# kakaobrain/rq-vae-transformer

Hardware: NVIDIA H100
Metric: 256x256 images/sec (ImageNet 1.4B RQ-Transformer, 8x8x4 codes, K=16384, top-k 1024, sample+decode) (higher is better)
Workload: dtype fp16

## Files before the change

### include/rqb200.h

```cpp
#ifndef RQB200_H
#define RQB200_H

#include <stddef.h>
#include <stdint.h>

#ifdef __cplusplus
extern "C" {
#endif

#define RQB200_OK 0
#define RQB200_EINVAL (-1)
#define RQB200_ECUDA (-2)
#define RQB200_ENODEV (-3)
#define RQB200_EWORKSPACE (-4)
#define RQB200_ESTATE (-5)

#define RQB200_F32 0
#define RQB200_BF16 1
#define RQB200_F16 2
#define RQB200_E4M3 3

#define RQB200_MODE_EXACT 0
#define RQB200_MODE_FAST 1

#define RQB200_AR_NO_GRAPH 1
#define RQB200_AR_NO_PDL 2
#define RQB200_AR_TRACE 4
#define RQB200_AR_SEQUENTIAL_PREFILL 32

const char* rqb200_last_error(void);
int rqb200_version(void);
int rqb200_device_count(void);

int rqb200_rq_quantize(const float* x, const float* codebook, int64_t N, int K, int C, int D, int64_t* codes,
                       float* quant_list, float* residual_out, void* stream);
int rqb200_rq_quantize_depthwise(const float* x, const float* const* codebooks_host, const int32_t* K_host, int64_t N, int C, int D,
                                 int64_t* codes, float* quant_list, float* residual_out, void* stream);

int rqb200_rq_soft_codes(const float* residual, const float* codebook, int64_t N, int K, int C, float temp, float* soft_out,
                         float* logits_out, void* stream);

int rqb200_rq_embed_sum(const int64_t* codes, const float* codebook, int64_t N, int D, int K, int C, float* out,
                        void* stream);
int rqb200_rq_embed_depth(const int64_t* codes, const float* codebook, int64_t N, int D, int K, int C, float* out,
                          void* stream);
int rqb200_rq_embed_sum_depthwise(const int64_t* codes, const float* const* codebooks_host, const int32_t* K_host, int64_t N, int D,
                                  int C, float* out, void* stream);
int rqb200_rq_embed_depth_depthwise(const int64_t* codes, const float* const* codebooks_host, const int32_t* K_host, int64_t N,
                                    int D, int C, float* out, void* stream);

int rqb200_sample_logits(const float* logits, const float* q, int B, int V, float temperature, int top_k,
                         float top_p, int64_t* out_idx, void* stream);

typedef struct rqb200_block_weights {
    const void *wqkv, *wproj, *w1, *w2;
    const float *bqkv, *bproj, *b1, *b2;
    const float *ln1_w, *ln1_b, *ln2_w, *ln2_b;
    const float *sqkv, *sproj, *s1, *s2;
} rqb200_block_weights;

typedef struct rqb200_ar_config {
    int32_t embed_dim, n_head, n_body, n_head_layers;
    int32_t vocab, H, W, D;
    int32_t vocab_cond, cond_len;
    int32_t code_dim, codebook_size;
    int32_t mode;
    int32_t weight_dtype;
    int32_t flags;
    int32_t split_qkv, split_proj, split_fc1, split_fc2;
    int32_t codebook_per_depth;
    int32_t embed_variant;
} rqb200_ar_config;

#define RQB200_EMB_TOK_INPUT 1
#define RQB200_EMB_TOK_HEAD 2
#define RQB200_EMB_NO_CUMSUM 4
#define RQB200_EMB_TUPLE 8
#define RQB200_EMB_CLS_PER_DEPTH 16

typedef struct rqb200_ar_weights {
    const float *pos_emb_cond, *pos_emb_hw, *pos_emb_d;
    const float* cond_emb;
    const void *w_in, *w_head, *w_cls;
    const float *b_in, *b_head, *b_cls;
    const float *cls_ln_w, *cls_ln_b;
    const float* codebook;
    const rqb200_block_weights* body;
    const rqb200_block_weights* head;
    const void* w_ccls;
    const float *b_ccls, *ccls_ln_w, *ccls_ln_b;
    const float* tok_emb;
    const float *s_in, *s_head, *s_cls, *s_ccls;
} rqb200_ar_weights;

typedef struct rqb200_ar rqb200_ar;

rqb200_ar* rqb200_ar_create(const rqb200_ar_config* cfg, const rqb200_ar_weights* w);
void rqb200_ar_destroy(rqb200_ar* h);
size_t rqb200_ar_workspace_bytes(const rqb200_ar* h, int B);

int rqb200_ar_sample(rqb200_ar* h, const int64_t* partial, const int64_t* cond, int B, int start_h, int start_w,
                     float temperature, const int32_t* top_k_host, const float* top_p_host, const float* noise,
                     int64_t noise_stride, float* logits_out, const int64_t* force_codes, int64_t* out_codes,
                     void* workspace, size_t workspace_bytes, void* stream);
int rqb200_ar_sample_span(rqb200_ar* h, const int64_t* partial, const int64_t* cond, int B, int idx_begin, int idx_end, int resume,
                          float temperature, const int32_t* top_k_host, const float* top_p_host, const float* noise,
                          int64_t noise_stride, float* logits_out, const int64_t* force_codes, int64_t* out_codes,
                          void* workspace, size_t workspace_bytes, void* stream);
int rqb200_ar_sample_span_cfg(rqb200_ar* h, const int64_t* partial, const int64_t* cond, int B, int idx_begin, int idx_end, int resume,
                              float temperature, const int32_t* top_k_host, const float* top_p_host, const float* noise,
                              int64_t noise_stride, float* logits_out, const int64_t* force_codes, int64_t* out_codes,
                              void* workspace, size_t workspace_bytes, void* stream, float cfg_scale);
int rqb200_ar_sample_span_keep(rqb200_ar* h, const int64_t* partial, const int64_t* cond, int B, int idx_begin, int idx_end, int resume,
                               float temperature, const int32_t* top_k_host, const float* top_p_host, const float* noise,
                               int64_t noise_stride, float* logits_out, const int64_t* force_codes, int64_t* out_codes,
                               void* workspace, size_t workspace_bytes, void* stream, const uint8_t* keep, const uint8_t* sampled_host,
                               int cfg_n, float cfg_scale);
int rqb200_ar_step(rqb200_ar* h, const int64_t* xs, int64_t xs_batch_stride, const int64_t* cond, int B, int pos_h, int pos_w,
                   int d, int restart, float* logits_out, void* workspace, size_t workspace_bytes, void* stream);
size_t rqb200_ar_forward_workspace_bytes(const rqb200_ar* h, int B);
int rqb200_ar_forward(rqb200_ar* h, const int64_t* codes, const int64_t* cond, int B, float* logits_out, float* cond_logits_out,
                      void* workspace, size_t workspace_bytes, void* stream);
size_t rqb200_ar_log_prob_workspace_bytes(const rqb200_ar* h, int B);
int rqb200_ar_log_prob(rqb200_ar* h, const int64_t* codes, const int64_t* cond, int B, float* logp_out, float* cond_logp_out,
                       void* workspace, size_t workspace_bytes, void* stream);
int rqb200_ar_trace(rqb200_ar* h, long long* out_host, int cap_launches, char* names, int names_cap);
int64_t rqb200_ar_last_launches(const rqb200_ar* h);

#define RQB200_VAE_NO_GN_FUSE 0x100
typedef struct rqb200_vae_config {
    int32_t ch, n_levels, ch_mult[8], num_res_blocks;
    int32_t n_attn_res, attn_resolutions[8];
    int32_t resolution, z_channels, embed_dim, in_channels, out_ch;
    int32_t codebook_size, depth;
    int32_t mode;
} rqb200_vae_config;

typedef struct rqb200_vae rqb200_vae;

rqb200_vae* rqb200_vae_create(const rqb200_vae_config* cfg);
void rqb200_vae_destroy(rqb200_vae* h);
int rqb200_vae_set_tensor(rqb200_vae* h, const char* key, const void* ptr, int dtype, int64_t numel);
int rqb200_vae_finalize(rqb200_vae* h);
size_t rqb200_vae_workspace_bytes(const rqb200_vae* h, int B);
int rqb200_vae_decode(rqb200_vae* h, const float* z_q, int B, float* out, void* workspace, size_t workspace_bytes,
                      void* stream);
int rqb200_vae_decode_code(rqb200_vae* h, const int64_t* codes, int B, float* out, void* workspace,
                           size_t workspace_bytes, void* stream);
int rqb200_vae_encode(rqb200_vae* h, const float* x, int B, float* z_e, void* workspace, size_t workspace_bytes,
                      void* stream);
int64_t rqb200_vae_last_launches(const rqb200_vae* h);

int rqb200_dbg_gemm_tc(const void* W16, const void* X16, const float* bias, const float* residual, void* out,
                       int out_is_16, int gelu, float* partial, int N_out, int K, int B, int splits, int fmt, void* stream);
int rqb200_dbg_gemm_tc_fp8(const void* W8_packed, const float* scale, const void* X16, const float* bias, const float* residual,
                           void* out, int out_is_16, int gelu, float* partial, int N_out, int K, int B, int splits, void* stream);

int rqb200_dbg_rq_quantize(int form, const float* x, const float* codebook, int64_t N, int K, int C, int D, int64_t* codes,
                           float* quant_list, float* residual_out, void* stream);
int rqb200_dbg_rq_quantize_depthwise(int form, const float* x, const float* const* codebooks_host, const int32_t* K_host, int64_t N,
                                     int C, int D, int64_t* codes, float* quant_list, float* residual_out, void* stream);
int rqb200_dbg_sample_logits(int algo, const float* logits, const float* q, int B, int V, float temperature, int top_k,
                             float top_p, int64_t* out_idx, void* stream);

int rqb200_dbg_conv_tc(const void* X16, const void* W16, const void* X16lo, const void* W16lo, const float* bias,
                       const float* residual, float* out, int B, int H, int W, int Cin, int Cout, int ks, int out_nchw,
                       void* stream);

int rqb200_dbg_conv_tc_gn(const void* X16, const void* W16, const void* X16lo, const void* W16lo, const float* bias,
                          const float* residual, float* out, double* gn_part, int B, int H, int W, int Cin, int Cout, int ks,
                          int out_nchw, void* stream);

int rqb200_dbg_rows_gemm(const void* X16, const void* W16, const float* bias, const float* residual, float* out_f32, void* out_16,
                         int gelu, int fmt, int64_t M, int N_out, int K, void* stream);

int rqb200_dbg_log_prob_rows(const float* logits, int64_t ld, int V, int64_t rows, const int64_t* targets, float* out, void* stream);

int rqb200_dbg_attn_step(int form, const float* part, int S, const float* bqkv, void* kc, void* vc, void* att, int B, int E, int Tmax,
                         const int* t_dev, int t_host, int fmt, void* stream);
int rqb200_dbg_prefill_attn(const void* qkv, void* kc, void* vc, void* att, int G, int T, int E, int Tmax, int fmt, void* stream);
int rqb200_dbg_append_attn(const void* qkv, void* kc, void* vc, void* att, int G, int T0, int T, int E, int Tmax, int fmt, void* stream);
int rqb200_dbg_ln(int form, const float* x_in, const float* part, int S, const float* bias, const float* extra, float* x_out, const float* g,
                  const float* b, void* xn, int64_t rows, int E, int fmt, void* stream);
int rqb200_dbg_act_reduce(const float* part, int S, const float* bias, void* h, int B, int N, int fmt, void* stream);

int rqb200_dbg_vae_conv(const float* X, const void* Wt, int wdtype, const float* bias, const float* residual, float* out, int B, int H,
                        int W, int Cin, int Cout, int ks, int stride, int upsample, int in_nchw, int out_nchw, void* stream);
int rqb200_dbg_groupnorm(int form, const float* X, const float* gamma, const float* beta, float* Y, void* Y16, void* Y16lo,
                         double* stats_ws, int64_t ws_doubles, int B, int HW, int C, int silu, void* stream);
int rqb200_dbg_cast_f16(const float* X, void* Y16, void* Y16lo, int B, int H, int W, int C, int upsample, void* stream);
int rqb200_dbg_vae_attn(const float* qkv, float* out, int B, int HW, int C, void* stream);

#ifdef __cplusplus
}
#endif
#endif
```

### rq-vae-transformer_b200/csrc/conv_tc.cu

```cuda
#include <cstdlib>

#include "kernels.h"
#include "tc_common.cuh"

namespace rqb {

struct ConvTcParams {
    int B, H, W, Cin, Cout;
    int ks;
    int stride;
    int TW, TH, NB;
    int tiles_x, tiles_y, tiles_b, n_tiles_n;
    const float* bias;
    const float* residual;
    float* out;
    int out_nchw;
    void* out16;
    int gelu, fmt;
    int64_t m_rows;
    double* gn_part;
    int gn_chunks;
};

constexpr int CT_THREADS = 288;
constexpr int CT_A_BYTES = 128 * 64 * 2;

template <int CG>
__device__ __forceinline__ void gn_chunk_stats(const float (&wv)[16], bool valid, int lane, float& tot, int& vidx, bool& writer) {
    constexpr int NG = 16 / CG, NV = 2 * NG;
    float vals[NV];
#pragma unroll
    for (int g = 0; g < NG; g++) {
        float s1 = 0.f, s2 = 0.f;
#pragma unroll
        for (int i = 0; i < CG; i++) {
            const float x = valid ? wv[g * CG + i] : 0.f;
            s1 += x;
            s2 = fmaf(x, x, s2);
        }
        vals[g] = s1;
        vals[NG + g] = s2;
    }
    int n = NV;
    vidx = 0;
    int keep_mask = 31;
#pragma unroll
    for (int S = 16; S >= 1; S >>= 1) {
        if (n > 1) {
            const int half = n >> 1;
            const bool up = (lane & S) != 0;
#pragma unroll
            for (int i = 0; i < NV / 2; i++)
                if (i < half) {
                    const float send = up ? vals[i] : vals[i + half];
                    const float keep = up ? vals[i + half] : vals[i];
                    vals[i] = keep + __shfl_xor_sync(0xffffffffu, send, S);
                }
            vidx += up ? half : 0;
            keep_mask &= ~S;
            n = half;
        } else {
            vals[0] += __shfl_xor_sync(0xffffffffu, vals[0], S);
        }
    }
    tot = vals[0];
    writer = (lane & keep_mask) == 0;
}

__device__ __forceinline__ void ct_epilogue16(const ConvTcParams& p, const float (&v)[16], int n0, int q, int lane, int tx, int ty, int tb,
                                              int b, int y, int x, int64_t pix, bool valid) {
    if (n0 >= p.Cout) return;
    if (p.out_nchw) {
        if (!valid) return;
#pragma unroll
        for (int i = 0; i < 16; i++) {
            const int n = n0 + i;
            if (n < p.Cout) p.out[(((int64_t)b * p.Cout + n) * p.H + y) * p.W + x] = v[i] + p.bias[n];
        }
    } else if (p.out16 != nullptr) {
        if (!valid) return;
        float w[16];
#pragma unroll
        for (int i = 0; i < 16; i += 4) {
            const float4 bb = *reinterpret_cast<const float4*>(p.bias + n0 + i);
            w[i] = v[i] + bb.x; w[i + 1] = v[i + 1] + bb.y; w[i + 2] = v[i + 2] + bb.z; w[i + 3] = v[i + 3] + bb.w;
        }
        if (p.gelu) {
#pragma unroll
            for (int i = 0; i < 16; i++) w[i] = gelu_erf(w[i]);
        }
        uint4 pk[2];
        uint32_t* pw = reinterpret_cast<uint32_t*>(pk);
#pragma unroll
        for (int i = 0; i < 8; i++) pw[i] = pack_h16x2(w[2 * i], w[2 * i + 1], p.fmt);
        uint4* o16 = reinterpret_cast<uint4*>(reinterpret_cast<h16*>(p.out16) + pix * p.Cout + n0);
        o16[0] = pk[0];
        o16[1] = pk[1];
    } else {
        float* o = p.out + pix * p.Cout + n0;
        const float* rs = p.residual ? p.residual + pix * p.Cout + n0 : nullptr;
        float wv[16];
#pragma unroll
        for (int i = 0; i < 16; i += 4) {
            float4 bb = *reinterpret_cast<const float4*>(p.bias + n0 + i);
            float4 w = make_float4(v[i] + bb.x, v[i + 1] + bb.y, v[i + 2] + bb.z, v[i + 3] + bb.w);
            if (rs && valid) {
                float4 rr = *reinterpret_cast<const float4*>(rs + i);
                w.x += rr.x; w.y += rr.y; w.z += rr.z; w.w += rr.w;
            }
            if (valid) *reinterpret_cast<float4*>(o + i) = w;
            wv[i] = w.x; wv[i + 1] = w.y; wv[i + 2] = w.z; wv[i + 3] = w.w;
        }
        if (p.gn_part != nullptr) {
            const int cg = p.Cout >> 5;
            const int wpi = (p.TW * p.TH) >> 5;
            const int chunk = (ty * p.tiles_x + tx) * wpi + (q % wpi);
            const int bw = tb * p.NB + (q * 32) / (p.TW * p.TH);
            float tot;
            int vidx;
            bool writer;
            if (cg == 4) gn_chunk_stats<4>(wv, valid, lane, tot, vidx, writer);
            else if (cg == 8) gn_chunk_stats<8>(wv, valid, lane, tot, vidx, writer);
            else gn_chunk_stats<16>(wv, valid, lane, tot, vidx, writer);
            const int ngr = 16 / cg;
            if (writer && bw < p.B)
                p.gn_part[(((int64_t)bw * p.gn_chunks + chunk) * 32 + (n0 / cg + (vidx % ngr))) * 2 + (vidx / ngr)] = (double)tot;
        }
    }
}

template <int BN, int FMT, int PASSES>
__device__ __forceinline__ void ct_mma_kblock(float (&acc)[BN / 2], uint32_t a, uint32_t b, bool first) {
    constexpr int B_BYTES = BN * 64 * 2;
    if (PASSES == 3) {
#pragma unroll
        for (int j = 0; j < 4; j++)
            tc::Wgmma<BN, FMT>::mma(acc, tc::gmma_desc_k128(a + CT_A_BYTES + j * 32), tc::gmma_desc_k128(b + j * 32),
                                    (!first || j > 0) ? 1u : 0u);
#pragma unroll
        for (int j = 0; j < 4; j++)
            tc::Wgmma<BN, FMT>::mma(acc, tc::gmma_desc_k128(a + j * 32), tc::gmma_desc_k128(b + B_BYTES + j * 32), 1u);
    }
#pragma unroll
    for (int j = 0; j < 4; j++)
        tc::Wgmma<BN, FMT>::mma(acc, tc::gmma_desc_k128(a + j * 32), tc::gmma_desc_k128(b + j * 32),
                                (PASSES == 3 || !first || j > 0) ? 1u : 0u);
}

template <int BN, int STAGES, int PASSES>
__global__ void __launch_bounds__(CT_THREADS, 1)
conv_tc_kernel(const __grid_constant__ CUtensorMap tmA, const __grid_constant__ CUtensorMap tmB,
               const __grid_constant__ CUtensorMap tmAlo, const __grid_constant__ CUtensorMap tmBlo, ConvTcParams p) {
    constexpr int B_BYTES = BN * 64 * 2;
    constexpr int NOPS = PASSES == 3 ? 2 : 1;
    constexpr int STAGE_BYTES = NOPS * (CT_A_BYTES + B_BYTES);
    constexpr int OFF_B = NOPS * CT_A_BYTES;
    constexpr int CW = BN < 32 ? BN : 32;
    extern __shared__ uint8_t smem_raw[];
    uint8_t* smem = reinterpret_cast<uint8_t*>((reinterpret_cast<uintptr_t>(smem_raw) + 1023) & ~uintptr_t(1023));
    float* stage = reinterpret_cast<float*>(smem + STAGES * STAGE_BYTES);
    uint64_t* full = reinterpret_cast<uint64_t*>(stage + 128 * (CW + 4));
    uint64_t* empty = full + STAGES;

    const int warp = threadIdx.x >> 5, lane = threadIdx.x & 31;
    const int cslabs = p.Cin / 64;
    const int nkb = p.ks * p.ks * cslabs;
    const int sx = p.stride;
    const int m_tiles = p.tiles_x * p.tiles_y * p.tiles_b;
    const int total = m_tiles * p.n_tiles_n;

    if (warp == 8 && lane == 0) {
        tc::prefetch_tmap(&tmA);
        tc::prefetch_tmap(&tmB);
        for (int s = 0; s < STAGES; s++) { tc::mbar_init(&full[s], 1); tc::mbar_init(&empty[s], 8); }
        tc::fence_barrier_init();
    }
    __syncthreads();

    if (warp == 8) {
        if (lane == 0) {
            uint32_t it = 0;
            for (int tile = blockIdx.x; tile < total; tile += gridDim.x) {
                const int nt = tile % p.n_tiles_n, mt = tile / p.n_tiles_n;
                const int tx = mt % p.tiles_x, ty = (mt / p.tiles_x) % p.tiles_y, tb = mt / (p.tiles_x * p.tiles_y);
                const int x0 = tx * p.TW, y0 = ty * p.TH, b0 = tb * p.NB;
                for (int kb = 0; kb < nkb; kb++, it++) {
                    const int s = it % STAGES;
                    tc::mbar_wait(&empty[s], ((it / STAGES) & 1) ^ 1);
                    const int tap = kb / cslabs, c0 = (kb % cslabs) * 64;
                    const int ky = tap / p.ks, kx = tap % p.ks;
                    tc::mbar_expect_tx(&full[s], STAGE_BYTES);
                    uint8_t* st = smem + s * STAGE_BYTES;
                    tc::tma_load_4d(st, &tmA, &full[s], c0, x0 * sx + kx, y0 * sx + ky, b0, tc::L2_EVICT_NORMAL);
                    tc::tma_load_2d(st + OFF_B, &tmB, &full[s], tap * p.Cin + c0, nt * BN, tc::L2_EVICT_LAST);
                    if (PASSES == 3) {
                        tc::tma_load_4d(st + CT_A_BYTES, &tmAlo, &full[s], c0, x0 * sx + kx, y0 * sx + ky, b0, tc::L2_EVICT_NORMAL);
                        tc::tma_load_2d(st + OFF_B + B_BYTES, &tmBlo, &full[s], tap * p.Cin + c0, nt * BN, tc::L2_EVICT_LAST);
                    }
                }
            }
        }
        return;
    }

    const int wg = warp >> 2, t = threadIdx.x;
    const int r = t & 127;
    const int rx = r % p.TW, ry = (r / p.TW) % p.TH, rb = r / (p.TW * p.TH);
    float acc[BN / 2];
#pragma unroll
    for (int i = 0; i < BN / 2; i++) acc[i] = 0.f;
    uint32_t it = 0;
    for (int tile = blockIdx.x; tile < total; tile += gridDim.x) {
        for (int kb = 0; kb < nkb; kb++, it++) {
            const int s = it % STAGES;
            tc::mbar_wait(&full[s], (it / STAGES) & 1);
            const uint32_t a = tc::smem_u32(smem + s * STAGE_BYTES) + wg * (64 * 128), b = tc::smem_u32(smem + s * STAGE_BYTES + OFF_B);
            tc::wgmma_fence();
            if (p.fmt) ct_mma_kblock<BN, 1, PASSES>(acc, a, b, kb == 0);
            else ct_mma_kblock<BN, 0, PASSES>(acc, a, b, kb == 0);
            tc::wgmma_commit();
            tc::wgmma_wait<1>();
            if (kb > 0 && lane == 0) tc::mbar_arrive(&empty[(it - 1) % STAGES]);
        }
        tc::wgmma_wait<0>();
        tc::acc_fence(acc);
        if (lane == 0) tc::mbar_arrive(&empty[(it - 1) % STAGES]);

        const int nt = tile % p.n_tiles_n, mt = tile / p.n_tiles_n;
        const int tx = mt % p.tiles_x, ty = (mt / p.tiles_x) % p.tiles_y, tb = mt / (p.tiles_x * p.tiles_y);
        const int x = tx * p.TW + rx, y = ty * p.TH + ry, b = tb * p.NB + rb;
        const int64_t pix = ((int64_t)b * p.H + y) * p.W + x;
        const bool valid = (x < p.W) && (y < p.H) && (b < p.B) && (p.m_rows == 0 || pix < p.m_rows);
        tc::drain_acc<BN, CW, 0>(acc, stage, wg, t, [&p, t, nt, tx, ty, tb, b, y, x, pix, valid](const float (&v)[16], int, int c) {
            ct_epilogue16(p, v, nt * BN + c, (t >> 5) & 3, t & 31, tx, ty, tb, b, y, x, pix, valid);
        });
    }
}

template <int BN, int STAGES, int PASSES>
static int launch_conv_tc_t(const CUtensorMap& tmA, const CUtensorMap& tmB, const CUtensorMap& tmAlo, const CUtensorMap& tmBlo,
                            const ConvTcParams& p, int n_sm, cudaStream_t st) {
    constexpr size_t smem = (size_t)STAGES * (PASSES == 3 ? 2 : 1) * (CT_A_BYTES + BN * 128) + 128 * ((BN < 32 ? BN : 32) + 4) * 4 + 1024 + 256;
    static_assert(smem <= 227 * 1024, "conv_tc: shared memory budget");
    RQB_ENSURE_SMEM(smem, conv_tc_kernel<BN, STAGES, PASSES>);
    const int total = p.tiles_x * p.tiles_y * p.tiles_b * p.n_tiles_n;
    const int grid = total < n_sm ? total : n_sm;
    conv_tc_kernel<BN, STAGES, PASSES><<<grid, CT_THREADS, smem, st>>>(tmA, tmB, tmAlo, tmBlo, p);
    return check_launch("conv_tc");
}

constexpr int C3_HALO_BYTES = 10 * 10 * 2 * 128;

template <int BN, int FMT, int PASSES>
__device__ __forceinline__ void c3_mma_kblock(float (&acc)[BN / 2], uint32_t a, uint32_t b, bool first) {
    constexpr int B_BYTES = BN * 64 * 2;
    constexpr uint32_t SBO = 10 * 128;
    if (PASSES == 3) {
#pragma unroll
        for (int j = 0; j < 4; j++)
            tc::Wgmma<BN, FMT>::mma(acc, tc::gmma_desc_k128(a + C3_HALO_BYTES + j * 32, SBO), tc::gmma_desc_k128(b + j * 32),
                                    (!first || j > 0) ? 1u : 0u);
#pragma unroll
        for (int j = 0; j < 4; j++)
            tc::Wgmma<BN, FMT>::mma(acc, tc::gmma_desc_k128(a + j * 32, SBO), tc::gmma_desc_k128(b + B_BYTES + j * 32), 1u);
    }
#pragma unroll
    for (int j = 0; j < 4; j++)
        tc::Wgmma<BN, FMT>::mma(acc, tc::gmma_desc_k128(a + j * 32, SBO), tc::gmma_desc_k128(b + j * 32),
                                (PASSES == 3 || !first || j > 0) ? 1u : 0u);
}

template <int BN, int STAGES, int PASSES>
__global__ void __launch_bounds__(CT_THREADS, 1)
conv3x3_tc_kernel(const __grid_constant__ CUtensorMap tmA, const __grid_constant__ CUtensorMap tmB,
                  const __grid_constant__ CUtensorMap tmAlo, const __grid_constant__ CUtensorMap tmBlo, ConvTcParams p) {
    constexpr int B_BYTES = BN * 64 * 2;
    constexpr int NOPS = PASSES == 3 ? 2 : 1;
    constexpr int HSLOTS = 2;
    constexpr int SLOT_BYTES = NOPS * C3_HALO_BYTES;
    constexpr int STAGE_BYTES = NOPS * B_BYTES;
    constexpr int CW = BN < 32 ? BN : 32;
    extern __shared__ uint8_t smem_raw[];
    uint8_t* smem = reinterpret_cast<uint8_t*>((reinterpret_cast<uintptr_t>(smem_raw) + 1023) & ~uintptr_t(1023));
    uint8_t* wst = smem + HSLOTS * SLOT_BYTES;
    float* stage = reinterpret_cast<float*>(wst + STAGES * STAGE_BYTES);
    uint64_t* full = reinterpret_cast<uint64_t*>(stage + 128 * (CW + 4));
    uint64_t* empty = full + STAGES;
    uint64_t* hfull = empty + STAGES;
    uint64_t* hempty = hfull + HSLOTS;

    const int warp = threadIdx.x >> 5, lane = threadIdx.x & 31;
    const int cslabs = p.Cin / 64;
    const int m_tiles = p.tiles_x * p.tiles_y * p.tiles_b;
    const int total = m_tiles * p.n_tiles_n;

    if (warp == 8 && lane == 0) {
        tc::prefetch_tmap(&tmA);
        tc::prefetch_tmap(&tmB);
        for (int s = 0; s < STAGES; s++) { tc::mbar_init(&full[s], 1); tc::mbar_init(&empty[s], 8); }
        for (int h = 0; h < HSLOTS; h++) { tc::mbar_init(&hfull[h], 1); tc::mbar_init(&hempty[h], 8); }
        tc::fence_barrier_init();
    }
    __syncthreads();

    if (warp == 8) {
        if (lane == 0) {
            const uint32_t halo_tx = NOPS * 10 * (p.TH + 2) * p.NB * 128;
            uint32_t it = 0, hit = 0;
            for (int tile = blockIdx.x; tile < total; tile += gridDim.x) {
                const int nt = tile % p.n_tiles_n, mt = tile / p.n_tiles_n;
                const int tx = mt % p.tiles_x, ty = (mt / p.tiles_x) % p.tiles_y, tb = mt / (p.tiles_x * p.tiles_y);
                const int x0 = tx * 8, y0 = ty * p.TH, b0 = tb * p.NB;
                for (int sl = 0; sl < cslabs; sl++, hit++) {
                    const int c0 = sl * 64;
                    for (int tap = 0; tap < 9; tap++, it++) {
                        const int s = it % STAGES;
                        tc::mbar_wait(&empty[s], ((it / STAGES) & 1) ^ 1);
                        tc::mbar_expect_tx(&full[s], STAGE_BYTES);
                        uint8_t* w = wst + s * STAGE_BYTES;
                        tc::tma_load_2d(w, &tmB, &full[s], tap * p.Cin + c0, nt * BN, tc::L2_EVICT_LAST);
                        if (PASSES == 3) tc::tma_load_2d(w + B_BYTES, &tmBlo, &full[s], tap * p.Cin + c0, nt * BN, tc::L2_EVICT_LAST);
                        if (tap == 0) {
                            const int h = hit % HSLOTS;
                            tc::mbar_wait(&hempty[h], ((hit / HSLOTS) & 1) ^ 1);
                            tc::mbar_expect_tx(&hfull[h], halo_tx);
                            uint8_t* a = smem + h * SLOT_BYTES;
                            tc::tma_load_4d(a, &tmA, &hfull[h], c0, x0 - 1, y0 - 1, b0, tc::L2_EVICT_NORMAL);
                            if (PASSES == 3) tc::tma_load_4d(a + C3_HALO_BYTES, &tmAlo, &hfull[h], c0, x0 - 1, y0 - 1, b0, tc::L2_EVICT_NORMAL);
                        }
                    }
                }
            }
        }
        return;
    }

    const int wg = warp >> 2, t = threadIdx.x;
    const int r = t & 127;
    const int rx = r % 8, ry = (r / 8) % p.TH, rb = r / (8 * p.TH);
    const uint32_t a_wg = (uint32_t)(((8 * wg / p.TH) * (p.TH + 2) + (8 * wg) % p.TH) * 10 * 128);
    float acc[BN / 2];
#pragma unroll
    for (int i = 0; i < BN / 2; i++) acc[i] = 0.f;
    uint32_t it = 0, hit = 0;
    for (int tile = blockIdx.x; tile < total; tile += gridDim.x) {
        for (int sl = 0; sl < cslabs; sl++, hit++) {
            const int h = hit % HSLOTS;
            tc::mbar_wait(&hfull[h], (hit / HSLOTS) & 1);
            const uint32_t a0 = tc::smem_u32(smem + h * SLOT_BYTES) + a_wg;
            for (int tap = 0; tap < 9; tap++, it++) {
                const int s = it % STAGES;
                tc::mbar_wait(&full[s], (it / STAGES) & 1);
                const uint32_t a = a0 + ((tap / 3) * 10 + tap % 3) * 128, b = tc::smem_u32(wst + s * STAGE_BYTES);
                const bool first = sl == 0 && tap == 0;
                tc::wgmma_fence();
                if (p.fmt) c3_mma_kblock<BN, 1, PASSES>(acc, a, b, first);
                else c3_mma_kblock<BN, 0, PASSES>(acc, a, b, first);
                tc::wgmma_commit();
                tc::wgmma_wait<1>();
                if (!first && lane == 0) {
                    tc::mbar_arrive(&empty[(it - 1) % STAGES]);
                    if (tap == 0) tc::mbar_arrive(&hempty[(hit - 1) % HSLOTS]);
                }
            }
        }
        tc::wgmma_wait<0>();
        tc::acc_fence(acc);
        if (lane == 0) {
            tc::mbar_arrive(&empty[(it - 1) % STAGES]);
            tc::mbar_arrive(&hempty[(hit - 1) % HSLOTS]);
        }

        const int nt = tile % p.n_tiles_n, mt = tile / p.n_tiles_n;
        const int tx = mt % p.tiles_x, ty = (mt / p.tiles_x) % p.tiles_y, tb = mt / (p.tiles_x * p.tiles_y);
        const int x = tx * 8 + rx, y = ty * p.TH + ry, b = tb * p.NB + rb;
        const int64_t pix = ((int64_t)b * p.H + y) * p.W + x;
        const bool valid = (x < p.W) && (y < p.H) && (b < p.B);
        tc::drain_acc<BN, CW, 0>(acc, stage, wg, t, [&p, t, nt, tx, ty, tb, b, y, x, pix, valid](const float (&v)[16], int, int c) {
            ct_epilogue16(p, v, nt * BN + c, (t >> 5) & 3, t & 31, tx, ty, tb, b, y, x, pix, valid);
        });
    }
}

template <int BN, int STAGES, int PASSES>
static int launch_conv3x3_tc_t(const CUtensorMap& tmA, const CUtensorMap& tmB, const CUtensorMap& tmAlo, const CUtensorMap& tmBlo,
                               const ConvTcParams& p, int n_sm, cudaStream_t st) {
    constexpr int NOPS = PASSES == 3 ? 2 : 1;
    constexpr size_t smem = (size_t)2 * NOPS * C3_HALO_BYTES + (size_t)STAGES * NOPS * BN * 128 +
                            128 * ((BN < 32 ? BN : 32) + 4) * 4 + 1024 + 256;
    static_assert(smem <= 227 * 1024, "conv3x3_tc: shared memory budget");
    RQB_ENSURE_SMEM(smem, conv3x3_tc_kernel<BN, STAGES, PASSES>);
    const int total = p.tiles_x * p.tiles_y * p.tiles_b * p.n_tiles_n;
    const int grid = total < n_sm ? total : n_sm;
    conv3x3_tc_kernel<BN, STAGES, PASSES><<<grid, CT_THREADS, smem, st>>>(tmA, tmB, tmAlo, tmBlo, p);
    return check_launch("conv3x3_tc");
}

static int sm_count() {
    static int n = 0;
    if (!n) {
        int dev = 0;
        cudaGetDevice(&dev);
        cudaDeviceGetAttribute(&n, cudaDevAttrMultiProcessorCount, dev);
        if (n <= 0) n = 132;
    }
    return n;
}

bool conv_tc_supported(int H, int W, int Cin, int Cout, int ks, int stride, int in_nchw) {
    if ((stride != 1 && !(stride == 2 && ks == 3)) || in_nchw || (ks != 1 && ks != 3)) return false;
    if (Cin % 64 != 0) return false;
    if (Cout != 3 && Cout % 128 != 0 && Cout != 64) return false;
    auto pow2 = [](int v) { return v > 0 && (v & (v - 1)) == 0; };
    return pow2(H) && pow2(W);
}

static void conv_tile(int H, int W, int ks, int stride, int& TW, int& TH, int& NB) {
    if (ks == 3 && stride == 1) {
        TW = 8;
        TH = H > 8 ? 16 : 8;
    } else {
        TW = W < 16 ? W : 16;
        TH = (128 / TW) < H ? (128 / TW) : H;
    }
    NB = 128 / (TW * TH);
}

bool conv_tc_gn_fusable(int H, int W, int Cout, int ks, int stride) {
    int TW, TH, NB;
    conv_tile(H, W, ks, stride, TW, TH, NB);
    const int cg = Cout / 32;
    return Cout % 32 == 0 && (cg == 4 || cg == 8 || cg == 16) && W % TW == 0 && H % TH == 0 && TW * TH >= 32 && (H * W) % 32 == 0;
}

int launch_conv_tc(const void* X16, const void* W16, const void* X16lo, const void* W16lo, const float* bias,
                   const float* residual, float* out, int B, int H, int W, int Cin, int Cout, int ks, int out_nchw,
                   cudaStream_t st, int stride, double* gn_part, int fmt) {
    ConvTcParams p = {};
    p.B = B; p.H = H; p.W = W; p.Cin = Cin; p.Cout = Cout; p.ks = ks; p.stride = stride; p.fmt = fmt;
    conv_tile(H, W, ks, stride, p.TW, p.TH, p.NB);
    if (p.TW * p.TH * p.NB != 128) return fail(RQB200_EINVAL, "conv_tc: feature map extent must be a power of two");
    p.tiles_x = (int)ceil_div(W, p.TW); p.tiles_y = (int)ceil_div(H, p.TH); p.tiles_b = (int)ceil_div(B, p.NB);
    const bool c3 = ks == 3 && stride == 1;
    const int BN = Cout <= 16 ? 16 : (Cout % 256 == 0 && !c3 ? 256 : (Cout % 128 == 0 ? 128 : 64));
    p.n_tiles_n = (int)ceil_div(Cout, BN);
    p.bias = bias; p.residual = residual; p.out = out; p.out_nchw = out_nchw;
    if (gn_part != nullptr) {
        if (!conv_tc_gn_fusable(H, W, Cout, ks, stride) || out_nchw)
            return fail(RQB200_EINVAL, "conv_tc: GroupNorm statistics cannot be fused for this shape");
        p.gn_part = gn_part;
        p.gn_chunks = H * W / 32;
    }
    const bool split = X16lo != nullptr && W16lo != nullptr;
    CUtensorMap tmA, tmB, tmAlo, tmBlo;
    RQB_TRY(make_tmap_2d(&tmB, W16, 1, (uint64_t)ks * ks * Cin, (uint64_t)Cout, (uint64_t)ks * ks * Cin * 2, 64, (uint32_t)BN));
    if (split)
        RQB_TRY(make_tmap_2d(&tmBlo, W16lo, 1, (uint64_t)ks * ks * Cin, (uint64_t)Cout, (uint64_t)ks * ks * Cin * 2, 64, (uint32_t)BN));
    const int n_sm = sm_count();
    if (c3) {
        RQB_TRY(make_tmap_4d_nhwc(&tmA, X16, (uint64_t)Cin, (uint64_t)W, (uint64_t)H, (uint64_t)B, 64, (uint32_t)p.TW + 2,
                                  (uint32_t)p.TH + 2, (uint32_t)p.NB, 1));
        if (split) {
            RQB_TRY(make_tmap_4d_nhwc(&tmAlo, X16lo, (uint64_t)Cin, (uint64_t)W, (uint64_t)H, (uint64_t)B, 64, (uint32_t)p.TW + 2,
                                      (uint32_t)p.TH + 2, (uint32_t)p.NB, 1));
            switch (BN) {
                case 16: return launch_conv3x3_tc_t<16, 8, 3>(tmA, tmB, tmAlo, tmBlo, p, n_sm, st);
                case 64: return launch_conv3x3_tc_t<64, 4, 3>(tmA, tmB, tmAlo, tmBlo, p, n_sm, st);
                default: return launch_conv3x3_tc_t<128, 3, 3>(tmA, tmB, tmAlo, tmBlo, p, n_sm, st);
            }
        }
        switch (BN) {
            case 16: return launch_conv3x3_tc_t<16, 8, 1>(tmA, tmB, tmA, tmB, p, n_sm, st);
            case 64: return launch_conv3x3_tc_t<64, 8, 1>(tmA, tmB, tmA, tmB, p, n_sm, st);
            default: return launch_conv3x3_tc_t<128, 8, 1>(tmA, tmB, tmA, tmB, p, n_sm, st);
        }
    }
    RQB_TRY(make_tmap_4d_nhwc(&tmA, X16, (uint64_t)Cin, (uint64_t)W * stride, (uint64_t)H * stride, (uint64_t)B, 64, (uint32_t)p.TW,
                              (uint32_t)p.TH, (uint32_t)p.NB, (uint32_t)stride));
    if (split) {
        RQB_TRY(make_tmap_4d_nhwc(&tmAlo, X16lo, (uint64_t)Cin, (uint64_t)W * stride, (uint64_t)H * stride, (uint64_t)B, 64,
                                  (uint32_t)p.TW, (uint32_t)p.TH, (uint32_t)p.NB, (uint32_t)stride));
        switch (BN) {
            case 16: return launch_conv_tc_t<16, 5, 3>(tmA, tmB, tmAlo, tmBlo, p, n_sm, st);
            case 64: return launch_conv_tc_t<64, 4, 3>(tmA, tmB, tmAlo, tmBlo, p, n_sm, st);
            case 128: return launch_conv_tc_t<128, 3, 3>(tmA, tmB, tmAlo, tmBlo, p, n_sm, st);
            default: return launch_conv_tc_t<256, 2, 3>(tmA, tmB, tmAlo, tmBlo, p, n_sm, st);
        }
    }
    switch (BN) {
        case 16: return launch_conv_tc_t<16, 8, 1>(tmA, tmB, tmA, tmB, p, n_sm, st);
        case 64: return launch_conv_tc_t<64, 8, 1>(tmA, tmB, tmA, tmB, p, n_sm, st);
        case 128: return launch_conv_tc_t<128, 6, 1>(tmA, tmB, tmA, tmB, p, n_sm, st);
        default: return launch_conv_tc_t<256, 4, 1>(tmA, tmB, tmA, tmB, p, n_sm, st);
    }
}

int launch_rows_gemm_tc(const void* X16, const void* W16, const float* bias, const float* residual, float* out_f32, void* out_16,
                        int gelu, int fmt, int64_t M, int N_out, int K, cudaStream_t st) {
    if (N_out % 128 != 0 || K % 64 != 0 || M < 1 || (out_f32 == nullptr) == (out_16 == nullptr) || bias == nullptr)
        return fail(RQB200_EINVAL, "rows_gemm_tc: need N_out % 128 == 0, K % 64 == 0, a bias and exactly one output");
    ConvTcParams p = {};
    p.B = (int)ceil_div(M, 128); p.H = 8; p.W = 16; p.Cin = K; p.Cout = N_out; p.ks = 1; p.stride = 1;
    p.TW = 16; p.TH = 8; p.NB = 1;
    p.tiles_x = 1; p.tiles_y = 1; p.tiles_b = p.B;
    const int BN = N_out % 256 == 0 ? 256 : 128;
    p.n_tiles_n = N_out / BN;
    p.bias = bias; p.residual = residual; p.out = out_f32; p.out_nchw = 0;
    p.out16 = out_16; p.gelu = gelu; p.fmt = fmt; p.m_rows = M;
    CUtensorMap tmA, tmB;
    RQB_TRY(make_tmap_4d_nhwc(&tmA, X16, (uint64_t)K, 16, 8, (uint64_t)p.B, 64, 16, 8, 1, 1));
    RQB_TRY(make_tmap_2d(&tmB, W16, 1, (uint64_t)K, (uint64_t)N_out, (uint64_t)K * 2, 64, (uint32_t)BN));
    const int n_sm = sm_count();
    if (BN == 256) return launch_conv_tc_t<256, 4, 1>(tmA, tmB, tmA, tmB, p, n_sm, st);
    return launch_conv_tc_t<128, 6, 1>(tmA, tmB, tmA, tmB, p, n_sm, st);
}

__device__ __forceinline__ void store_split4(__half* hi, __half* lo, const float (&v)[4]) {
    __half2 h0 = __floats2half2_rn(v[0], v[1]), h1 = __floats2half2_rn(v[2], v[3]);
    uint2 pk;
    pk.x = *reinterpret_cast<uint32_t*>(&h0);
    pk.y = *reinterpret_cast<uint32_t*>(&h1);
    *reinterpret_cast<uint2*>(hi) = pk;
    if (lo) {
        float2 f0 = __half22float2(h0), f1 = __half22float2(h1);
        __half2 l0 = __floats2half2_rn(v[0] - f0.x, v[1] - f0.y), l1 = __floats2half2_rn(v[2] - f1.x, v[3] - f1.y);
        pk.x = *reinterpret_cast<uint32_t*>(&l0);
        pk.y = *reinterpret_cast<uint32_t*>(&l1);
        *reinterpret_cast<uint2*>(lo) = pk;
    }
}

__global__ void gn_finalize_kernel(double* __restrict__ part, int B, int nchunks, double n, double eps) {
    const int i = (blockIdx.x * blockDim.x + threadIdx.x) >> 5, lane = threadIdx.x & 31;
    if (i >= B * 32) return;
    const int b = i / 32, g = i % 32;
    double ts = 0.0, tss = 0.0;
    for (int c = lane; c < nchunks; c += 32) {
        const double* o = part + (((int64_t)b * nchunks + c) * 32 + g) * 2;
        ts += o[0];
        tss += o[1];
    }
    ts = warp_sum_d(ts);
    tss = warp_sum_d(tss);
    if (lane != 0) return;
    double mean = ts / n, var = tss / n - mean * mean;
    if (var < 0.0) var = 0.0;
    double* fin = part + (int64_t)B * nchunks * 64 + (int64_t)i * 2;
    fin[0] = mean;
    fin[1] = 1.0 / sqrt(var + eps);
}

__global__ void __launch_bounds__(256) gn_apply_f16_kernel(const float* __restrict__ X, const double* __restrict__ part,
                                                           const float* __restrict__ gamma, const float* __restrict__ beta,
                                                           __half* __restrict__ Y, __half* __restrict__ Ylo, int HW, int C,
                                                           float eps, int silu, int nchunks) {
    __shared__ float s_mean[32], s_rstd[32];
    const int b = blockIdx.y;
    const int cg = C / 32;
    if (threadIdx.x < 32) {
        const double* fin = part + (int64_t)gridDim.y * nchunks * 64 + ((int64_t)b * 32 + threadIdx.x) * 2;
        s_mean[threadIdx.x] = (float)fin[0];
        s_rstd[threadIdx.x] = (float)fin[1];
    }
    __syncthreads();
    (void)eps;
    const int c8n = C / 8;
    const unsigned total8 = (unsigned)HW * (unsigned)c8n;
    const float* Xb = X + (int64_t)b * HW * C;
    __half* Yb = Y + (int64_t)b * HW * C;
    __half* Lb = Ylo ? Ylo + (int64_t)b * HW * C : nullptr;
    for (unsigned i = blockIdx.x * 256u + threadIdx.x; i < total8; i += gridDim.x * 256u) {
        const int c = (int)(i % (unsigned)c8n) * 8;
        const float4 x0 = __ldcs(reinterpret_cast<const float4*>(Xb + (size_t)i * 8));
        const float4 x1 = __ldcs(reinterpret_cast<const float4*>(Xb + (size_t)i * 8 + 4));
        const float4 ga0 = *reinterpret_cast<const float4*>(gamma + c), ga1 = *reinterpret_cast<const float4*>(gamma + c + 4);
        const float4 be0 = *reinterpret_cast<const float4*>(beta + c), be1 = *reinterpret_cast<const float4*>(beta + c + 4);
        const int g0 = c / cg, g1 = (c + 4) / cg;
        const float m0 = s_mean[g0], r0 = s_rstd[g0], m1 = s_mean[g1], r1 = s_rstd[g1];
        float v[8] = {(x0.x - m0) * r0 * ga0.x + be0.x, (x0.y - m0) * r0 * ga0.y + be0.y, (x0.z - m0) * r0 * ga0.z + be0.z,
                      (x0.w - m0) * r0 * ga0.w + be0.w, (x1.x - m1) * r1 * ga1.x + be1.x, (x1.y - m1) * r1 * ga1.y + be1.y,
                      (x1.z - m1) * r1 * ga1.z + be1.z, (x1.w - m1) * r1 * ga1.w + be1.w};
        if (silu) {
#pragma unroll
            for (int k = 0; k < 8; k++) v[k] = v[k] / (1.0f + __expf(-v[k]));
        }
        __half2 h[4], l[4];
#pragma unroll
        for (int k = 0; k < 4; k++) {
            h[k] = __floats2half2_rn(v[2 * k], v[2 * k + 1]);
            const float2 f = __half22float2(h[k]);
            l[k] = __floats2half2_rn(v[2 * k] - f.x, v[2 * k + 1] - f.y);
        }
        *reinterpret_cast<uint4*>(Yb + (size_t)i * 8) = *reinterpret_cast<uint4*>(h);
        if (Lb) *reinterpret_cast<uint4*>(Lb + (size_t)i * 8) = *reinterpret_cast<uint4*>(l);
    }
}

__global__ void __launch_bounds__(256) cast_f16_kernel(const float* __restrict__ X, __half* __restrict__ Y, __half* __restrict__ Ylo,
                                                       int B, int H, int W, int C, int upsample) {
    const int c4n = C / 4;
    const int Ho = upsample ? 2 * H : H, Wo = upsample ? 2 * W : W;
    const int64_t total4 = (int64_t)B * Ho * Wo * c4n;
    for (int64_t i = (int64_t)blockIdx.x * 256 + threadIdx.x; i < total4; i += (int64_t)gridDim.x * 256) {
        const int c4 = (int)(i % c4n);
        int64_t pix = i / c4n;
        const int ox = (int)(pix % Wo), oy = (int)((pix / Wo) % Ho), b = (int)(pix / ((int64_t)Wo * Ho));
        const int ix = upsample ? ox >> 1 : ox, iy = upsample ? oy >> 1 : oy;
        const float4 x = *reinterpret_cast<const float4*>(X + (((int64_t)b * H + iy) * W + ix) * C + c4 * 4);
        const float v[4] = {x.x, x.y, x.z, x.w};
        store_split4(Y + i * 4, Ylo ? Ylo + i * 4 : nullptr, v);
    }
}

int launch_groupnorm_f16(const float* X, const float* gamma, const float* beta, void* Y16, void* Y16lo, double* stats_ws, int B,
                         int HW, int C, int silu, cudaStream_t st, int fused_chunks) {
    if (C % 128 != 0) return fail(RQB200_EINVAL, "groupnorm_f16: C % 128 != 0");
    const int nchunks = fused_chunks > 0 ? fused_chunks : (int)ceil_div(HW, 256);
    if (fused_chunks <= 0) RQB_TRY(launch_gn_stats(X, stats_ws, B, HW, C, st));
    gn_finalize_kernel<<<(unsigned)ceil_div(B * 32 * 32, 128), 128, 0, st>>>(stats_ws, B, nchunks, (double)HW * (C / 32), 1e-6);
    RQB_TRY(check_launch("gn_finalize"));
    int gx = (int)std::min<int64_t>(ceil_div((int64_t)HW * C / 8, 256), 1024);
    gn_apply_f16_kernel<<<dim3(gx, B), 256, 0, st>>>(X, stats_ws, gamma, beta, (__half*)Y16, (__half*)Y16lo, HW, C, 1e-6f, silu, nchunks);
    return check_launch("gn_apply_f16");
}

int launch_cast_f16(const float* X, void* Y16, void* Y16lo, int B, int H, int W, int C, int upsample, cudaStream_t st) {
    if (C % 4 != 0) return fail(RQB200_EINVAL, "cast_f16: C % 4 != 0");
    int64_t total4 = (int64_t)B * H * W * C / 4 * (upsample ? 4 : 1);
    int gx = (int)std::min<int64_t>(ceil_div(total4, 256), sm_count() * 16);
    cast_f16_kernel<<<gx, 256, 0, st>>>(X, (__half*)Y16, (__half*)Y16lo, B, H, W, C, upsample);
    return check_launch("cast_f16");
}

}

extern "C" int rqb200_dbg_conv_tc(const void* X16, const void* W16, const void* X16lo, const void* W16lo, const float* bias,
                                  const float* residual, float* out, int B, int H, int W, int Cin, int Cout, int ks, int out_nchw,
                                  void* stream) {
    const int stride = (out_nchw >> 8) > 1 ? (out_nchw >> 8) : 1;
    if (!rqb::conv_tc_supported(H, W, Cin, Cout, ks, stride, 0)) return rqb::fail(RQB200_EINVAL, "conv_tc: unsupported shape");
    return rqb::launch_conv_tc(X16, W16, X16lo, W16lo, bias, residual, out, B, H, W, Cin, Cout, ks, out_nchw & 1, (cudaStream_t)stream,
                               stride, nullptr, (out_nchw >> 1) & 1);
}

extern "C" int rqb200_dbg_conv_tc_gn(const void* X16, const void* W16, const void* X16lo, const void* W16lo, const float* bias,
                                     const float* residual, float* out, double* gn_part, int B, int H, int W, int Cin, int Cout, int ks,
                                     int out_nchw, void* stream) {
    const int stride = (out_nchw >> 8) > 1 ? (out_nchw >> 8) : 1;
    if (!rqb::conv_tc_supported(H, W, Cin, Cout, ks, stride, 0)) return rqb::fail(RQB200_EINVAL, "conv_tc: unsupported shape");
    return rqb::launch_conv_tc(X16, W16, X16lo, W16lo, bias, residual, out, B, H, W, Cin, Cout, ks, out_nchw & 1, (cudaStream_t)stream,
                               stride, gn_part, (out_nchw >> 1) & 1);
}

extern "C" int rqb200_dbg_rows_gemm(const void* X16, const void* W16, const float* bias, const float* residual, float* out_f32,
                                    void* out_16, int gelu, int fmt, int64_t M, int N_out, int K, void* stream) {
    return rqb::launch_rows_gemm_tc(X16, W16, bias, residual, out_f32, out_16, gelu, fmt, M, N_out, K, (cudaStream_t)stream);
}
```

### rq-vae-transformer_b200/csrc/kernels.h

```cpp
#pragma once
#include <cuda.h>

#include "common.cuh"

namespace rqb {
constexpr int RQ_MAX_TABLES = 16;
struct RqTables {
    const float* cb[RQ_MAX_TABLES];
    int K[RQ_MAX_TABLES];
    int n;
    __host__ __device__ __forceinline__ int of(int depth) const { return n == 1 ? 0 : depth; }
};
int make_rq_tables(RqTables* out, const float* const* cb_host, const int32_t* K_host, int n);

int launch_rq_quantize(const float* x, const RqTables& tabs, int64_t N, int C, int D, int64_t* codes, float* quant_list,
                       float* resid_out, cudaStream_t st, int form = 0);
bool rq_quantize2_supported(int64_t N, const RqTables& tabs, int C);
int launch_rq_quantize2(const float* x, const RqTables& tabs, int64_t N, int C, int D, int64_t* codes, float* quant_list,
                        float* resid_out, cudaStream_t st);
int launch_rq_embed(const int64_t* codes, const RqTables& tabs, int64_t N, int D, int C, float* out, bool sum, cudaStream_t st);
int launch_sample(const float* logits, const float* q, int B, int V, float temperature, int top_k, float top_p,
                  int64_t* out_idx, const int64_t* force, int64_t out_stride, cudaStream_t st, int algo = 1, int cfg_n = 0,
                  float cfg_s = 0.f, const uint8_t* keep = nullptr);
int launch_logprob_rows(const float* lg, int64_t ld, int V, int64_t rows, const int64_t* tgt, int64_t tgt_stride, float* out,
                        cudaStream_t st);
int launch_gather_targets(const int64_t* src, int A1, int A2, int G, int64_t sa, int64_t sc, int64_t sg, int64_t off, int64_t* dst,
                          cudaStream_t st);
int launch_linear(const float* X, int64_t ldx, const void* W, int wdtype, const float* bias, const float* R, float* Y,
                  int64_t ldy, int M, int N, int K, int act, cudaStream_t st);
int launch_layernorm(const float* X, int64_t ldx, const float* g, const float* b, float* Y, int64_t ldy, int M, int E,
                     cudaStream_t st);
int launch_attn_cached(const float* qkv, float* kc, float* vc, float* out, int B, int Tn, int T_past, int Tmax, int E,
                       int nh, cudaStream_t st);
int launch_code_emb(const int64_t* codes, const float* cb, int64_t cb_dstride, int B, int HW, int D, int K, int C, int j0, int J,
                    float* out, cudaStream_t st);
int launch_body_token(const float* lin, const float* pos_hw, int B, int D, int E, int j0, int J, int s0, int Tn, float* X,
                      cudaStream_t st);
int launch_cond_token(const int64_t* cond, const float* cond_emb, const float* pos_cond, int B, int cond_len, int vocab_cond,
                      int E, int Tn, float* X, cudaStream_t st);
int launch_head_cumsum(const int64_t* codes, const float* cb, int64_t cb_dstride, int B, int HW, int D, int K, int C, int j, int d,
                       float* out, cudaStream_t st, bool last_only = false);
int launch_row_add(const float* in, int64_t in_row_stride, int64_t in_off, const float* pos, int B, int E, float* out,
                   cudaStream_t st);
struct ConvGeom {
    int B, Hi, Wi, Cin;
    int Ho, Wo, Cout;
    int KH, KW, stride;
    int pad;
    int upsample;
    int out_nchw;
    int in_nchw;
};
ConvGeom vae_conv_geom(int B, int H, int W, int Cin, int Cout, int ks, int stride, int upsample, int in_nchw, int out_nchw);
int launch_conv(const float* X, const void* W, int wdtype, const float* bias, const float* R, float* Y, const ConvGeom& g,
                cudaStream_t st);
int launch_groupnorm_silu(const float* X, const float* gamma, const float* beta, float* Y, double* stats_ws, int B, int HW,
                          int C, int silu, cudaStream_t st);
int launch_vae_attn(const float* qkv, float* out, int B, int HW, int C, cudaStream_t st);
size_t groupnorm_ws_doubles(int B, int HW);
int launch_gn_stats(const float* X, double* stats_ws, int B, int HW, int C, cudaStream_t st);
bool conv_tc_supported(int H, int W, int Cin, int Cout, int ks, int stride, int in_nchw);
int launch_conv_tc(const void* X16, const void* W16, const void* X16lo, const void* W16lo, const float* bias,
                   const float* residual, float* out, int B, int H, int W, int Cin, int Cout, int ks, int out_nchw,
                   cudaStream_t st, int stride = 1, double* gn_part = nullptr, int fmt = 0);
bool conv_tc_gn_fusable(int H, int W, int Cout, int ks, int stride);
int launch_rows_gemm_tc(const void* X16, const void* W16, const float* bias, const float* residual, float* out_f32, void* out_16,
                        int gelu, int fmt, int64_t M, int N_out, int K, cudaStream_t st);
int launch_groupnorm_f16(const float* X, const float* gamma, const float* beta, void* Y16, void* Y16lo, double* stats_ws, int B,
                         int HW, int C, int silu, cudaStream_t st, int fused_chunks = 0);
int launch_cast_f16(const float* X, void* Y16, void* Y16lo, int B, int H, int W, int C, int upsample, cudaStream_t st);
int make_tmap_4d_nhwc(CUtensorMap* out, const void* base, uint64_t C, uint64_t W, uint64_t H, uint64_t B, uint32_t box_c,
                      uint32_t box_w, uint32_t box_h, uint32_t box_b, uint32_t stride = 1);

enum GemmTcMode { GT_F32 = 0, GT_H16 = 1, GT_H16_GELU = 2, GT_PARTIAL = 3 };
struct GemmTcParams {
    int N_out, K, B, splits, mode;
    int fmt;
    const float* bias;
    float bias_scale;
    const float* residual;
    int64_t ld_res, res_row_stride;
    const int* res_row_ptr;
    int res_div;
    void* out;
    int64_t ld_out;
    float* partial;
    long long* trace;
};
struct StreamedWeight {
    int N_out = 0, K = 0;
    const void* w16 = nullptr;
    CUtensorMap tm;
    const uint8_t* q8 = nullptr;
    const float* s8 = nullptr;
    bool e4m3() const { return w16 == nullptr; }
};
int make_streamed_weight(StreamedWeight* out, bool e4m3, const void* w, const float* scale, int N_out, int K);
inline int gemm_tc_chunk_rows(const StreamedWeight& w, int64_t rows) {
    return rows <= 16 ? 16 : rows <= 32 ? 32 : rows <= 64 ? 64 : (rows <= 128 || w.e4m3()) ? 128 : 256;
}
int launch_gemm_tc(const StreamedWeight& w, const CUtensorMap& tmX, GemmTcParams p, bool pdl, cudaStream_t st);
int make_tmap_2d(CUtensorMap* out, const void* base, int elem_bytes_log2, uint64_t inner, uint64_t outer,
                 uint64_t row_stride_bytes, uint32_t box_inner, uint32_t box_outer);

struct StepState {
    int s;
    int idx;
    int step;
    int cfg_n;
    const int64_t* cond;
    int64_t* codes;
    const int64_t* force;
    const float* noise;
    float* logits_out;
    int64_t noise_stride;
    float temperature;
    float cfg_scale;
    const uint8_t* keep;
    int top_k[8];
    float top_p[8];
};

inline bool plan_sampled(const uint8_t* sampled, int p) { return sampled == nullptr || sampled[p] != 0; }
inline int plan_prev(const uint8_t* sampled, int p) {
    for (int i = p - 1; i >= 0; i--)
        if (plan_sampled(sampled, i)) return i;
    return -1;
}
int launch_sample_dyn(const float* logits, const StepState* stt, int d, int B, int V, int HW, int D, cudaStream_t st, bool pdl);

struct ArFast;
ArFast* ar_fast_create(const rqb200_ar_config& cfg, const rqb200_ar_weights& w, const rqb200_block_weights* body,
                       const rqb200_block_weights* head);
void ar_fast_destroy(ArFast* f);
size_t ar_fast_workspace_bytes(const ArFast* f, int B);
int ar_fast_sample(ArFast* f, const int64_t* partial, const int64_t* cond, int B, int idx_begin, int idx_end, int resume,
                   float temperature, const int32_t* top_k, const float* top_p, const float* noise, int64_t noise_stride,
                   float* logits_out, const int64_t* force, int64_t* out, void* wsp, size_t ws_bytes, cudaStream_t st, int cfg_n,
                   float cfg_s, const uint8_t* keep, const uint8_t* sampled);
int ar_fast_step(ArFast* f, const int64_t* xs, int64_t xs_stride, const int64_t* cond, int B, int idx, int d, int restart,
                 float* logits_out, void* wsp, size_t ws_bytes, cudaStream_t st);
size_t ar_fast_forward_workspace_bytes(const ArFast* f, int B);
int ar_fast_forward(ArFast* f, const int64_t* codes, const int64_t* cond, int B, float* logits_out, float* cond_logits_out, void* wsp,
                    size_t ws_bytes, cudaStream_t st);
size_t ar_fast_log_prob_workspace_bytes(const ArFast* f, int B);
int ar_fast_log_prob(ArFast* f, const int64_t* codes, const int64_t* cond, int B, float* logp_out, float* cond_logp_out, void* wsp,
                     size_t ws_bytes, cudaStream_t st);
int ar_fast_trace(ArFast* f, long long* out_host, int cap_launches, char* names, int names_cap);
}
```

### rq-vae-transformer_b200/csrc/vae_engine.cu

```cuda
#include <string>
#include <unordered_map>
#include <vector>

#include "kernels.h"

struct VTensor {
    const void* ptr;
    int dtype;
    int64_t numel;
};

struct rqb200_vae {
    rqb200_vae_config cfg;
    std::unordered_map<std::string, VTensor> t;
    bool finalized = false;
    bool fast_ok = false;
    bool split = false;
    bool enc_fast = false;
    bool gn_fuse = true;
    int64_t last_launches = 0;
    int64_t max_act = 0;
    int64_t max_gn_hw = 0;
    rqb::RqTables codebooks{};
};

namespace rqb {

struct Operand {
    const float* x;
    int slot;
    int upsample;
    int nchw;
};

struct VaeRun {
    rqb200_vae* h;
    cudaStream_t st;
    int B;
    bool dry;
    float* buf[4];
    double* gn_ws;
    std::string missing;
    __half* h16[2] = {nullptr, nullptr};
    __half* l16[2] = {nullptr, nullptr};
    float* zq = nullptr;
    bool fast = false;

    const float* stats_buf = nullptr;
    int stats_chunks = 0;

    const VTensor* get(const std::string& k, int64_t numel) {
        auto it = h->t.find(k);
        if (it == h->t.end() || it->second.numel != numel) {
            if (missing.empty()) missing = k + (it == h->t.end() ? " (missing)" : " (wrong size)");
            return nullptr;
        }
        return &it->second;
    }
    void note_act(int64_t hw, int64_t c) { if (hw * c > h->max_act) h->max_act = hw * c; }

    int operand(const float* x, int H, int W, int C, int slot, int upsample, Operand* o) {
        *o = fast ? Operand{nullptr, slot, upsample, 0} : Operand{x, -1, upsample, 0};
        if (!fast || dry) return 0;
        return launch_cast_f16(x, h16[slot], l16[slot], B, H, W, C, upsample, st);
    }
    int norm(const std::string& name, const float* in, float* out, int HW, int C, int silu, Operand* o) {
        const VTensor* g = get(name + ".weight", C);
        const VTensor* b = get(name + ".bias", C);
        if (HW > h->max_gn_hw) h->max_gn_hw = HW;
        note_act(HW, C);
        *o = fast ? Operand{nullptr, 0, 0, 0} : Operand{out, -1, 0, 0};
        if (dry || !g || !b) return 0;
        if (!fast) return launch_groupnorm_silu(in, (const float*)g->ptr, (const float*)b->ptr, out, gn_ws, B, HW, C, silu, st);
        const int fused = (in == stats_buf) ? stats_chunks : 0;
        stats_buf = nullptr;
        return launch_groupnorm_f16(in, (const float*)g->ptr, (const float*)b->ptr, h16[0], l16[0], gn_ws, B, HW, C, silu, st, fused);
    }
    int conv(const std::string& name, const Operand& in, float* out, const float* resid, int H, int W, int Cin, int Cout, int ks,
             int stride, bool feeds_gn, int out_nchw) {
        const ConvGeom g = vae_conv_geom(B, H, W, Cin, Cout, ks, stride, in.upsample, in.nchw, out_nchw);
        const int Ho = g.Ho, Wo = g.Wo;
        const VTensor* w = get(name + ".weight", (int64_t)Cout * ks * ks * Cin);
        const VTensor* b = get(name + ".bias", Cout);
        note_act((int64_t)Ho * Wo, Cout);
        if (dry || !w || !b) return 0;
        if (in.slot < 0) return launch_conv(in.x, w->ptr, w->dtype, (const float*)b->ptr, resid, out, g, st);
        if (w->dtype != RQB200_F16) return fail(RQB200_ESTATE, "vae fast tier: conv weights must be fp16: " + name);
        const __half* in_lo = nullptr;
        const void* w_lo = nullptr;
        if (h->split) {
            const VTensor* wl = get(name + ".weight_lo", (int64_t)Cout * ks * ks * Cin);
            if (!wl) return 0;
            w_lo = wl->ptr;
            in_lo = l16[in.slot];
        }
        const bool fuse = feeds_gn && h->gn_fuse && !out_nchw && conv_tc_gn_fusable(Ho, Wo, Cout, ks, stride);
        stats_buf = fuse ? out : nullptr;
        stats_chunks = fuse ? Ho * Wo / 32 : 0;
        return launch_conv_tc(h16[in.slot], w->ptr, in_lo, w_lo, (const float*)b->ptr, resid, out, B, Ho, Wo, Cin, Cout, ks, out_nchw, st,
                              stride, fuse ? gn_ws : nullptr);
    }

    int resblock(const std::string& p, int& cur, int H, int W, int Cin, int Cout) {
        const int a = (cur + 1) & 3, b = (cur + 2) & 3, c = (cur + 3) & 3;
        Operand x;
        RQB_TRY(norm(p + ".norm1", buf[cur], buf[a], H * W, Cin, 1, &x));
        RQB_TRY(conv(p + ".conv1", x, buf[b], nullptr, H, W, Cin, Cout, 3, 1, true, 0));
        RQB_TRY(norm(p + ".norm2", buf[b], buf[a], H * W, Cout, 1, &x));
        const float* res = buf[cur];
        if (Cin != Cout) {
            Operand s;
            RQB_TRY(operand(buf[cur], H, W, Cin, 1, 0, &s));
            RQB_TRY(conv(p + ".nin_shortcut", s, buf[c], nullptr, H, W, Cin, Cout, 1, 1, false, 0));
            res = buf[c];
        }
        RQB_TRY(conv(p + ".conv2", x, buf[b], res, H, W, Cout, Cout, 3, 1, true, 0));
        cur = b;
        return 0;
    }
    int attnblock(const std::string& p, int& cur, int H, int W, int C) {
        const int a = (cur + 1) & 3, b = (cur + 2) & 3, c = (cur + 3) & 3;
        Operand x;
        RQB_TRY(norm(p + ".norm", buf[cur], buf[a], H * W, C, 0, &x));
        RQB_TRY(conv(p + ".qkv", x, buf[b], nullptr, H, W, C, 3 * C, 1, 1, false, 0));
        if (!dry && missing.empty()) RQB_TRY(launch_vae_attn(buf[b], buf[a], B, H * W, C, st));
        RQB_TRY(operand(buf[a], H, W, C, 0, 0, &x));
        RQB_TRY(conv(p + ".proj_out", x, buf[c], buf[cur], H, W, C, C, 1, 1, true, 0));
        cur = c;
        return 0;
    }
    bool has_attn(int res) const {
        for (int i = 0; i < h->cfg.n_attn_res; i++) if (h->cfg.attn_resolutions[i] == res) return true;
        return false;
    }

    int decode(const float* z, float* out) {
        fast = h->fast_ok;
        const rqb200_vae_config& c = h->cfg;
        const int nl = c.n_levels, nb = c.num_res_blocks;
        int res = c.resolution >> (nl - 1), ch = c.ch * c.ch_mult[nl - 1], cur = 0;
        Operand x;
        RQB_TRY(operand(z, res, res, c.embed_dim, 0, 0, &x));
        RQB_TRY(conv("post_quant_conv", x, buf[1], nullptr, res, res, c.embed_dim, c.z_channels, 1, 1, false, 0));
        RQB_TRY(operand(buf[1], res, res, c.z_channels, 0, 0, &x));
        RQB_TRY(conv("decoder.conv_in", x, buf[0], nullptr, res, res, c.z_channels, ch, 3, 1, true, 0));
        RQB_TRY(resblock("decoder.mid.block_1", cur, res, res, ch, ch));
        RQB_TRY(attnblock("decoder.mid.attn_1", cur, res, res, ch));
        RQB_TRY(resblock("decoder.mid.block_2", cur, res, res, ch, ch));
        for (int lvl = nl - 1; lvl >= 0; lvl--) {
            const int cout = c.ch * c.ch_mult[lvl];
            const std::string p = "decoder.up." + std::to_string(lvl);
            for (int b = 0; b <= nb; b++) {
                RQB_TRY(resblock(p + ".block." + std::to_string(b), cur, res, res, ch, cout));
                ch = cout;
                if (has_attn(res)) RQB_TRY(attnblock(p + ".attn." + std::to_string(b), cur, res, res, ch));
            }
            if (lvl != 0) {
                const int nxt = (cur + 1) & 3;
                RQB_TRY(operand(buf[cur], res, res, ch, 1, 1, &x));
                RQB_TRY(conv(p + ".upsample.conv", x, buf[nxt], nullptr, res, res, ch, ch, 3, 1, true, 0));
                cur = nxt;
                res *= 2;
            }
        }
        RQB_TRY(norm("decoder.norm_out", buf[cur], buf[(cur + 1) & 3], res * res, ch, 1, &x));
        return conv("decoder.conv_out", x, out, nullptr, res, res, ch, c.out_ch, 3, 1, false, 1);
    }

    int encode(const float* x, float* z_e) {
        fast = h->fast_ok && h->enc_fast;
        const rqb200_vae_config& c = h->cfg;
        const int nl = c.n_levels, nb = c.num_res_blocks;
        int res = c.resolution, ch = c.ch, cur = 0;
        RQB_TRY(conv("encoder.conv_in", Operand{x, -1, 0, 1}, buf[0], nullptr, res, res, c.in_channels, ch, 3, 1, false, 0));
        Operand o;
        for (int lvl = 0; lvl < nl; lvl++) {
            const int cout = c.ch * c.ch_mult[lvl];
            const std::string p = "encoder.down." + std::to_string(lvl);
            for (int b = 0; b < nb; b++) {
                RQB_TRY(resblock(p + ".block." + std::to_string(b), cur, res, res, ch, cout));
                ch = cout;
                if (has_attn(res)) RQB_TRY(attnblock(p + ".attn." + std::to_string(b), cur, res, res, ch));
            }
            if (lvl != nl - 1) {
                const int nxt = (cur + 1) & 3;
                RQB_TRY(operand(buf[cur], res, res, ch, 1, 0, &o));
                RQB_TRY(conv(p + ".downsample.conv", o, buf[nxt], nullptr, res, res, ch, ch, 3, 2, true, 0));
                cur = nxt;
                res /= 2;
            }
        }
        RQB_TRY(resblock("encoder.mid.block_1", cur, res, res, ch, ch));
        RQB_TRY(attnblock("encoder.mid.attn_1", cur, res, res, ch));
        RQB_TRY(resblock("encoder.mid.block_2", cur, res, res, ch, ch));
        float* zc = buf[(cur + 2) & 3];
        RQB_TRY(norm("encoder.norm_out", buf[cur], buf[(cur + 1) & 3], res * res, ch, 1, &o));
        RQB_TRY(conv("encoder.conv_out", o, zc, nullptr, res, res, ch, c.z_channels, 3, 1, false, 0));
        RQB_TRY(operand(zc, res, res, c.z_channels, 0, 0, &o));
        return conv("quant_conv", o, z_e, nullptr, res, res, c.z_channels, c.embed_dim, 1, 1, false, 0);
    }
};

static size_t vae_layout(const rqb200_vae* h, int B, void* base, size_t cap, VaeRun* run) {
    Arena a(base, cap);
    for (int i = 0; i < 4; i++) {
        float* p = a.take<float>((size_t)B * h->max_act);
        if (run) run->buf[i] = p;
    }
    double* g = a.take<double>(groupnorm_ws_doubles(B, (int)h->max_gn_hw));
    if (run) run->gn_ws = g;
    const rqb200_vae_config& c = h->cfg;
    int r = c.resolution >> (c.n_levels - 1);
    float* zq = a.take<float>((size_t)B * r * r * c.embed_dim);
    if (run) run->zq = zq;
    for (int i = 0; i < 2; i++) {
        __half* p16 = a.take<__half>((size_t)B * h->max_act);
        if (run) run->h16[i] = p16;
    }
    if (h->split)
        for (int i = 0; i < 2; i++) {
            __half* p16 = a.take<__half>((size_t)B * h->max_act);
            if (run) run->l16[i] = p16;
        }
    return a.off + 256;
}

}

extern "C" {

rqb200_vae* rqb200_vae_create(const rqb200_vae_config* cfg) {
    if (!cfg || cfg->n_levels < 1 || cfg->n_levels > 8 || cfg->n_attn_res > 8) { rqb::set_error("vae_create: bad config"); return nullptr; }
    rqb200_vae* h = new rqb200_vae();
    h->cfg = *cfg;
    return h;
}
void rqb200_vae_destroy(rqb200_vae* h) { delete h; }

int rqb200_vae_set_tensor(rqb200_vae* h, const char* key, const void* ptr, int dtype, int64_t numel) {
    if (!h || !key || !ptr) return rqb::fail(RQB200_EINVAL, "vae_set_tensor: null argument");
    h->t[key] = VTensor{ptr, dtype, numel};
    h->finalized = false;
    return 0;
}

int rqb200_vae_finalize(rqb200_vae* h) {
    if (!h) return rqb::fail(RQB200_EINVAL, "vae_finalize: null handle");
    rqb::VaeRun run{h, nullptr, 1, true, {nullptr, nullptr, nullptr, nullptr}, nullptr, ""};
    h->max_act = 0;
    h->max_gn_hw = 0;
    {
        const rqb200_vae_config& c = h->cfg;
        int r = c.resolution >> (c.n_levels - 1);
        bool ok = (c.mode & 0xff) == RQB200_MODE_FAST && c.ch % 128 == 0 && c.z_channels % 128 == 0 && c.embed_dim % 128 == 0 &&
                  c.out_ch == 3 && r > 0 && (r & (r - 1)) == 0;
        h->fast_ok = ok;
        h->gn_fuse = !(c.mode & RQB200_VAE_NO_GN_FUSE);
        h->split = ok && h->t.find("decoder.conv_in.weight_lo") != h->t.end();
    }
    {
        auto it = h->t.find("encoder.conv_out.weight");
        h->enc_fast = h->fast_ok && it != h->t.end() && it->second.dtype == RQB200_F16;
    }
    run.decode(nullptr, nullptr);
    run.encode(nullptr, nullptr);
    if (!run.missing.empty()) return rqb::fail(RQB200_ESTATE, "vae_finalize: tensor " + run.missing);
    {
        const rqb200_vae_config& c = h->cfg;
        const bool shared = h->t.count("codebook") != 0, per_depth = h->t.count("codebook.0") != 0;
        if (!shared && !per_depth) return rqb::fail(RQB200_ESTATE, "vae_finalize: tensor codebook (missing)");
        if (shared && per_depth) return rqb::fail(RQB200_EINVAL, "vae_finalize: both codebook and codebook.<d> registered");
        if (per_depth && (c.depth < 1 || c.depth > rqb::RQ_MAX_TABLES))
            return rqb::fail(RQB200_EINVAL, "vae_finalize: per-depth codebooks need depth 1..16");
        const float* ptrs[rqb::RQ_MAX_TABLES];
        int32_t ks[rqb::RQ_MAX_TABLES];
        const int n = shared ? 1 : c.depth;
        for (int d = 0; d < n; d++) {
            auto it = h->t.find(shared ? std::string("codebook") : "codebook." + std::to_string(d));
            if (it == h->t.end()) return rqb::fail(RQB200_ESTATE, "vae_finalize: tensor codebook." + std::to_string(d) + " (missing)");
            ptrs[d] = (const float*)it->second.ptr;
            ks[d] = shared ? c.codebook_size : (int32_t)(it->second.numel / c.embed_dim);
            if (!shared && (int64_t)ks[d] * c.embed_dim != it->second.numel)
                return rqb::fail(RQB200_EINVAL, "vae_finalize: codebook." + std::to_string(d) + " is not [K, embed_dim]");
        }
        RQB_TRY(rqb::make_rq_tables(&h->codebooks, ptrs, ks, n));
    }
    h->finalized = true;
    return 0;
}

size_t rqb200_vae_workspace_bytes(const rqb200_vae* h, int B) {
    if (!h || !h->finalized || B <= 0) return 0;
    return rqb::vae_layout(h, B, nullptr, 0, nullptr);
}

static int vae_prepare(rqb200_vae* h, int B, void* ws, size_t ws_bytes, void* stream, rqb::VaeRun* run) {
    if (!h || !ws) return rqb::fail(RQB200_EINVAL, "vae: null argument");
    if (!h->finalized) return rqb::fail(RQB200_ESTATE, "vae: engine not finalised");
    if (B <= 0) return rqb::fail(RQB200_EINVAL, "vae: B must be > 0");
    if (rqb200_device_count() <= 0) return rqb::fail(RQB200_ENODEV, "vae: no CUDA device");
    *run = rqb::VaeRun{h, (cudaStream_t)stream, B, false, {nullptr, nullptr, nullptr, nullptr}, nullptr, ""};
    size_t need = rqb::vae_layout(h, B, ws, ws_bytes, run);
    if (need > ws_bytes) return rqb::fail(RQB200_EWORKSPACE, "vae: workspace too small");
    rqb::g_launches = 0;
    return 0;
}

int rqb200_vae_decode(rqb200_vae* h, const float* z_q, int B, float* out, void* workspace, size_t workspace_bytes,
                      void* stream) {
    rqb::VaeRun run;
    RQB_TRY(vae_prepare(h, B, workspace, workspace_bytes, stream, &run));
    int rc = run.decode(z_q, out);
    h->last_launches = rqb::g_launches;
    return rc;
}

int rqb200_vae_decode_code(rqb200_vae* h, const int64_t* codes, int B, float* out, void* workspace,
                           size_t workspace_bytes, void* stream) {
    rqb::VaeRun run;
    RQB_TRY(vae_prepare(h, B, workspace, workspace_bytes, stream, &run));
    const rqb200_vae_config& c = h->cfg;
    int r = c.resolution >> (c.n_levels - 1);
    RQB_TRY(rqb::launch_rq_embed(codes, h->codebooks, (int64_t)B * r * r, c.depth, c.embed_dim, run.zq, true, (cudaStream_t)stream));
    int rc = run.decode(run.zq, out);
    h->last_launches = rqb::g_launches;
    return rc;
}

int rqb200_vae_encode(rqb200_vae* h, const float* x, int B, float* z_e, void* workspace, size_t workspace_bytes,
                      void* stream) {
    rqb::VaeRun run;
    RQB_TRY(vae_prepare(h, B, workspace, workspace_bytes, stream, &run));
    int rc = run.encode(x, z_e);
    h->last_launches = rqb::g_launches;
    return rc;
}
int64_t rqb200_vae_last_launches(const rqb200_vae* h) { return h ? h->last_launches : 0; }


int rqb200_dbg_vae_conv(const float* X, const void* Wt, int wdtype, const float* bias, const float* residual, float* out, int B, int H,
                        int W, int Cin, int Cout, int ks, int stride, int upsample, int in_nchw, int out_nchw, void* stream) {
    using namespace rqb;
    if (B < 1 || H < 1 || W < 1 || Cin < 1 || Cout < 1 || (ks != 1 && ks != 3) || (stride != 1 && stride != 2) || (upsample && stride != 1))
        return fail(RQB200_EINVAL, "dbg_vae_conv: need B, H, W, Cin, Cout >= 1, ks 1 | 3, stride 1 | 2, no upsample with stride 2");
    if (!X || !Wt || !out || (residual && out_nchw)) return fail(RQB200_EINVAL, "dbg_vae_conv: null argument, or a residual with NCHW output");
    if (rqb200_device_count() <= 0) return fail(RQB200_ENODEV, "dbg_vae_conv: no CUDA device");
    const ConvGeom g = vae_conv_geom(B, H, W, Cin, Cout, ks, stride, upsample != 0, in_nchw != 0, out_nchw != 0);
    return launch_conv(X, Wt, wdtype, bias, residual, out, g, (cudaStream_t)stream);
}

int rqb200_dbg_groupnorm(int form, const float* X, const float* gamma, const float* beta, float* Y, void* Y16, void* Y16lo,
                         double* stats_ws, int64_t ws_doubles, int B, int HW, int C, int silu, void* stream) {
    using namespace rqb;
    if (form < 0 || form > 2 || B < 1 || HW < 1 || C < 32 || C % 32 || (form > 0 && C % 128) || (form == 2 && HW % 32))
        return fail(RQB200_EINVAL, "dbg_groupnorm: need form 0..2, B, HW >= 1, C % 32 == 0 (forms 1, 2: C % 128 == 0; form 2: HW % 32 == 0)");
    if (!X || !gamma || !beta || !stats_ws || (form == 0 ? !Y : !Y16))
        return fail(RQB200_EINVAL, "dbg_groupnorm: null argument");
    if (ws_doubles < 0 || (size_t)ws_doubles < groupnorm_ws_doubles(B, HW))
        return fail(RQB200_EWORKSPACE, "dbg_groupnorm: statistics workspace smaller than groupnorm_ws_doubles(B, HW)");
    if (rqb200_device_count() <= 0) return fail(RQB200_ENODEV, "dbg_groupnorm: no CUDA device");
    const cudaStream_t st = (cudaStream_t)stream;
    if (form == 0) return launch_groupnorm_silu(X, gamma, beta, Y, stats_ws, B, HW, C, silu != 0, st);
    return launch_groupnorm_f16(X, gamma, beta, Y16, Y16lo, stats_ws, B, HW, C, silu != 0, st, form == 2 ? HW / 32 : 0);
}

int rqb200_dbg_cast_f16(const float* X, void* Y16, void* Y16lo, int B, int H, int W, int C, int upsample, void* stream) {
    using namespace rqb;
    if (B < 1 || H < 1 || W < 1 || C < 4) return fail(RQB200_EINVAL, "dbg_cast_f16: need B, H, W >= 1, C >= 4");
    if (!X || !Y16) return fail(RQB200_EINVAL, "dbg_cast_f16: null argument");
    if (rqb200_device_count() <= 0) return fail(RQB200_ENODEV, "dbg_cast_f16: no CUDA device");
    return launch_cast_f16(X, Y16, Y16lo, B, H, W, C, upsample != 0, (cudaStream_t)stream);
}

int rqb200_dbg_vae_attn(const float* qkv, float* out, int B, int HW, int C, void* stream) {
    using namespace rqb;
    if (B < 1 || HW < 1 || C < 1) return fail(RQB200_EINVAL, "dbg_vae_attn: need B, HW, C >= 1");
    if (!qkv || !out) return fail(RQB200_EINVAL, "dbg_vae_attn: null argument");
    if (rqb200_device_count() <= 0) return fail(RQB200_ENODEV, "dbg_vae_attn: no CUDA device");
    return launch_vae_attn(qkv, out, B, HW, C, (cudaStream_t)stream);
}
}
```

### rq-vae-transformer_b200/csrc/wgmma.cuh

```cuda
#pragma once
#include <stdint.h>

namespace rqb {
namespace tc {

template <int N, int FMT>
struct Wgmma;

template <>
struct Wgmma<16, 0> {
    static __device__ __forceinline__ void mma(float (&d)[8], uint64_t da, uint64_t db, uint32_t accumulate) {
        asm volatile(
            "{\n"
            ".reg .pred p;\n"
            "setp.ne.b32 p, %10, 0;\n"
            "wgmma.mma_async.sync.aligned.m64n16k16.f32.f16.f16 {%0, %1, %2, %3, %4, %5, %6, %7}, %8, %9, p, 1, 1, 0, 0;\n"
            "}\n"
            : "+f"(d[0]), "+f"(d[1]), "+f"(d[2]), "+f"(d[3]), "+f"(d[4]), "+f"(d[5]), "+f"(d[6]), "+f"(d[7])
            : "l"(da), "l"(db), "r"(accumulate));
    }
};

template <>
struct Wgmma<32, 0> {
    static __device__ __forceinline__ void mma(float (&d)[16], uint64_t da, uint64_t db, uint32_t accumulate) {
        asm volatile(
            "{\n"
            ".reg .pred p;\n"
            "setp.ne.b32 p, %18, 0;\n"
            "wgmma.mma_async.sync.aligned.m64n32k16.f32.f16.f16 {%0, %1, %2, %3, %4, %5, %6, %7, %8, %9, %10, %11, %12, %13, %14, %15}, %16, %17, p, 1, 1, 0, 0;\n"
            "}\n"
            : "+f"(d[0]), "+f"(d[1]), "+f"(d[2]), "+f"(d[3]), "+f"(d[4]), "+f"(d[5]), "+f"(d[6]), "+f"(d[7]), "+f"(d[8]), "+f"(d[9]), "+f"(d[10]), "+f"(d[11]), "+f"(d[12]), "+f"(d[13]), "+f"(d[14]), "+f"(d[15])
            : "l"(da), "l"(db), "r"(accumulate));
    }
};

template <>
struct Wgmma<64, 0> {
    static __device__ __forceinline__ void mma(float (&d)[32], uint64_t da, uint64_t db, uint32_t accumulate) {
        asm volatile(
            "{\n"
            ".reg .pred p;\n"
            "setp.ne.b32 p, %34, 0;\n"
            "wgmma.mma_async.sync.aligned.m64n64k16.f32.f16.f16 {%0, %1, %2, %3, %4, %5, %6, %7, %8, %9, %10, %11, %12, %13, %14, %15, %16, %17, %18, %19, %20, %21, %22, %23, %24, %25, %26, %27, %28, %29, %30, %31}, %32, %33, p, 1, 1, 0, 0;\n"
            "}\n"
            : "+f"(d[0]), "+f"(d[1]), "+f"(d[2]), "+f"(d[3]), "+f"(d[4]), "+f"(d[5]), "+f"(d[6]), "+f"(d[7]), "+f"(d[8]), "+f"(d[9]), "+f"(d[10]), "+f"(d[11]), "+f"(d[12]), "+f"(d[13]), "+f"(d[14]), "+f"(d[15]), "+f"(d[16]), "+f"(d[17]), "+f"(d[18]), "+f"(d[19]), "+f"(d[20]), "+f"(d[21]), "+f"(d[22]), "+f"(d[23]), "+f"(d[24]), "+f"(d[25]), "+f"(d[26]), "+f"(d[27]), "+f"(d[28]), "+f"(d[29]), "+f"(d[30]), "+f"(d[31])
            : "l"(da), "l"(db), "r"(accumulate));
    }
};

template <>
struct Wgmma<128, 0> {
    static __device__ __forceinline__ void mma(float (&d)[64], uint64_t da, uint64_t db, uint32_t accumulate) {
        asm volatile(
            "{\n"
            ".reg .pred p;\n"
            "setp.ne.b32 p, %66, 0;\n"
            "wgmma.mma_async.sync.aligned.m64n128k16.f32.f16.f16 {%0, %1, %2, %3, %4, %5, %6, %7, %8, %9, %10, %11, %12, %13, %14, %15, %16, %17, %18, %19, %20, %21, %22, %23, %24, %25, %26, %27, %28, %29, %30, %31, %32, %33, %34, %35, %36, %37, %38, %39, %40, %41, %42, %43, %44, %45, %46, %47, %48, %49, %50, %51, %52, %53, %54, %55, %56, %57, %58, %59, %60, %61, %62, %63}, %64, %65, p, 1, 1, 0, 0;\n"
            "}\n"
            : "+f"(d[0]), "+f"(d[1]), "+f"(d[2]), "+f"(d[3]), "+f"(d[4]), "+f"(d[5]), "+f"(d[6]), "+f"(d[7]), "+f"(d[8]), "+f"(d[9]), "+f"(d[10]), "+f"(d[11]), "+f"(d[12]), "+f"(d[13]), "+f"(d[14]), "+f"(d[15]), "+f"(d[16]), "+f"(d[17]), "+f"(d[18]), "+f"(d[19]), "+f"(d[20]), "+f"(d[21]), "+f"(d[22]), "+f"(d[23]), "+f"(d[24]), "+f"(d[25]), "+f"(d[26]), "+f"(d[27]), "+f"(d[28]), "+f"(d[29]), "+f"(d[30]), "+f"(d[31]), "+f"(d[32]), "+f"(d[33]), "+f"(d[34]), "+f"(d[35]), "+f"(d[36]), "+f"(d[37]), "+f"(d[38]), "+f"(d[39]), "+f"(d[40]), "+f"(d[41]), "+f"(d[42]), "+f"(d[43]), "+f"(d[44]), "+f"(d[45]), "+f"(d[46]), "+f"(d[47]), "+f"(d[48]), "+f"(d[49]), "+f"(d[50]), "+f"(d[51]), "+f"(d[52]), "+f"(d[53]), "+f"(d[54]), "+f"(d[55]), "+f"(d[56]), "+f"(d[57]), "+f"(d[58]), "+f"(d[59]), "+f"(d[60]), "+f"(d[61]), "+f"(d[62]), "+f"(d[63])
            : "l"(da), "l"(db), "r"(accumulate));
    }
};

template <>
struct Wgmma<256, 0> {
    static __device__ __forceinline__ void mma(float (&d)[128], uint64_t da, uint64_t db, uint32_t accumulate) {
        asm volatile(
            "{\n"
            ".reg .pred p;\n"
            "setp.ne.b32 p, %130, 0;\n"
            "wgmma.mma_async.sync.aligned.m64n256k16.f32.f16.f16 {%0, %1, %2, %3, %4, %5, %6, %7, %8, %9, %10, %11, %12, %13, %14, %15, %16, %17, %18, %19, %20, %21, %22, %23, %24, %25, %26, %27, %28, %29, %30, %31, %32, %33, %34, %35, %36, %37, %38, %39, %40, %41, %42, %43, %44, %45, %46, %47, %48, %49, %50, %51, %52, %53, %54, %55, %56, %57, %58, %59, %60, %61, %62, %63, %64, %65, %66, %67, %68, %69, %70, %71, %72, %73, %74, %75, %76, %77, %78, %79, %80, %81, %82, %83, %84, %85, %86, %87, %88, %89, %90, %91, %92, %93, %94, %95, %96, %97, %98, %99, %100, %101, %102, %103, %104, %105, %106, %107, %108, %109, %110, %111, %112, %113, %114, %115, %116, %117, %118, %119, %120, %121, %122, %123, %124, %125, %126, %127}, %128, %129, p, 1, 1, 0, 0;\n"
            "}\n"
            : "+f"(d[0]), "+f"(d[1]), "+f"(d[2]), "+f"(d[3]), "+f"(d[4]), "+f"(d[5]), "+f"(d[6]), "+f"(d[7]), "+f"(d[8]), "+f"(d[9]), "+f"(d[10]), "+f"(d[11]), "+f"(d[12]), "+f"(d[13]), "+f"(d[14]), "+f"(d[15]), "+f"(d[16]), "+f"(d[17]), "+f"(d[18]), "+f"(d[19]), "+f"(d[20]), "+f"(d[21]), "+f"(d[22]), "+f"(d[23]), "+f"(d[24]), "+f"(d[25]), "+f"(d[26]), "+f"(d[27]), "+f"(d[28]), "+f"(d[29]), "+f"(d[30]), "+f"(d[31]), "+f"(d[32]), "+f"(d[33]), "+f"(d[34]), "+f"(d[35]), "+f"(d[36]), "+f"(d[37]), "+f"(d[38]), "+f"(d[39]), "+f"(d[40]), "+f"(d[41]), "+f"(d[42]), "+f"(d[43]), "+f"(d[44]), "+f"(d[45]), "+f"(d[46]), "+f"(d[47]), "+f"(d[48]), "+f"(d[49]), "+f"(d[50]), "+f"(d[51]), "+f"(d[52]), "+f"(d[53]), "+f"(d[54]), "+f"(d[55]), "+f"(d[56]), "+f"(d[57]), "+f"(d[58]), "+f"(d[59]), "+f"(d[60]), "+f"(d[61]), "+f"(d[62]), "+f"(d[63]), "+f"(d[64]), "+f"(d[65]), "+f"(d[66]), "+f"(d[67]), "+f"(d[68]), "+f"(d[69]), "+f"(d[70]), "+f"(d[71]), "+f"(d[72]), "+f"(d[73]), "+f"(d[74]), "+f"(d[75]), "+f"(d[76]), "+f"(d[77]), "+f"(d[78]), "+f"(d[79]), "+f"(d[80]), "+f"(d[81]), "+f"(d[82]), "+f"(d[83]), "+f"(d[84]), "+f"(d[85]), "+f"(d[86]), "+f"(d[87]), "+f"(d[88]), "+f"(d[89]), "+f"(d[90]), "+f"(d[91]), "+f"(d[92]), "+f"(d[93]), "+f"(d[94]), "+f"(d[95]), "+f"(d[96]), "+f"(d[97]), "+f"(d[98]), "+f"(d[99]), "+f"(d[100]), "+f"(d[101]), "+f"(d[102]), "+f"(d[103]), "+f"(d[104]), "+f"(d[105]), "+f"(d[106]), "+f"(d[107]), "+f"(d[108]), "+f"(d[109]), "+f"(d[110]), "+f"(d[111]), "+f"(d[112]), "+f"(d[113]), "+f"(d[114]), "+f"(d[115]), "+f"(d[116]), "+f"(d[117]), "+f"(d[118]), "+f"(d[119]), "+f"(d[120]), "+f"(d[121]), "+f"(d[122]), "+f"(d[123]), "+f"(d[124]), "+f"(d[125]), "+f"(d[126]), "+f"(d[127])
            : "l"(da), "l"(db), "r"(accumulate));
    }
};

template <>
struct Wgmma<16, 1> {
    static __device__ __forceinline__ void mma(float (&d)[8], uint64_t da, uint64_t db, uint32_t accumulate) {
        asm volatile(
            "{\n"
            ".reg .pred p;\n"
            "setp.ne.b32 p, %10, 0;\n"
            "wgmma.mma_async.sync.aligned.m64n16k16.f32.bf16.bf16 {%0, %1, %2, %3, %4, %5, %6, %7}, %8, %9, p, 1, 1, 0, 0;\n"
            "}\n"
            : "+f"(d[0]), "+f"(d[1]), "+f"(d[2]), "+f"(d[3]), "+f"(d[4]), "+f"(d[5]), "+f"(d[6]), "+f"(d[7])
            : "l"(da), "l"(db), "r"(accumulate));
    }
};

template <>
struct Wgmma<32, 1> {
    static __device__ __forceinline__ void mma(float (&d)[16], uint64_t da, uint64_t db, uint32_t accumulate) {
        asm volatile(
            "{\n"
            ".reg .pred p;\n"
            "setp.ne.b32 p, %18, 0;\n"
            "wgmma.mma_async.sync.aligned.m64n32k16.f32.bf16.bf16 {%0, %1, %2, %3, %4, %5, %6, %7, %8, %9, %10, %11, %12, %13, %14, %15}, %16, %17, p, 1, 1, 0, 0;\n"
            "}\n"
            : "+f"(d[0]), "+f"(d[1]), "+f"(d[2]), "+f"(d[3]), "+f"(d[4]), "+f"(d[5]), "+f"(d[6]), "+f"(d[7]), "+f"(d[8]), "+f"(d[9]), "+f"(d[10]), "+f"(d[11]), "+f"(d[12]), "+f"(d[13]), "+f"(d[14]), "+f"(d[15])
            : "l"(da), "l"(db), "r"(accumulate));
    }
};

template <>
struct Wgmma<64, 1> {
    static __device__ __forceinline__ void mma(float (&d)[32], uint64_t da, uint64_t db, uint32_t accumulate) {
        asm volatile(
            "{\n"
            ".reg .pred p;\n"
            "setp.ne.b32 p, %34, 0;\n"
            "wgmma.mma_async.sync.aligned.m64n64k16.f32.bf16.bf16 {%0, %1, %2, %3, %4, %5, %6, %7, %8, %9, %10, %11, %12, %13, %14, %15, %16, %17, %18, %19, %20, %21, %22, %23, %24, %25, %26, %27, %28, %29, %30, %31}, %32, %33, p, 1, 1, 0, 0;\n"
            "}\n"
            : "+f"(d[0]), "+f"(d[1]), "+f"(d[2]), "+f"(d[3]), "+f"(d[4]), "+f"(d[5]), "+f"(d[6]), "+f"(d[7]), "+f"(d[8]), "+f"(d[9]), "+f"(d[10]), "+f"(d[11]), "+f"(d[12]), "+f"(d[13]), "+f"(d[14]), "+f"(d[15]), "+f"(d[16]), "+f"(d[17]), "+f"(d[18]), "+f"(d[19]), "+f"(d[20]), "+f"(d[21]), "+f"(d[22]), "+f"(d[23]), "+f"(d[24]), "+f"(d[25]), "+f"(d[26]), "+f"(d[27]), "+f"(d[28]), "+f"(d[29]), "+f"(d[30]), "+f"(d[31])
            : "l"(da), "l"(db), "r"(accumulate));
    }
};

template <>
struct Wgmma<128, 1> {
    static __device__ __forceinline__ void mma(float (&d)[64], uint64_t da, uint64_t db, uint32_t accumulate) {
        asm volatile(
            "{\n"
            ".reg .pred p;\n"
            "setp.ne.b32 p, %66, 0;\n"
            "wgmma.mma_async.sync.aligned.m64n128k16.f32.bf16.bf16 {%0, %1, %2, %3, %4, %5, %6, %7, %8, %9, %10, %11, %12, %13, %14, %15, %16, %17, %18, %19, %20, %21, %22, %23, %24, %25, %26, %27, %28, %29, %30, %31, %32, %33, %34, %35, %36, %37, %38, %39, %40, %41, %42, %43, %44, %45, %46, %47, %48, %49, %50, %51, %52, %53, %54, %55, %56, %57, %58, %59, %60, %61, %62, %63}, %64, %65, p, 1, 1, 0, 0;\n"
            "}\n"
            : "+f"(d[0]), "+f"(d[1]), "+f"(d[2]), "+f"(d[3]), "+f"(d[4]), "+f"(d[5]), "+f"(d[6]), "+f"(d[7]), "+f"(d[8]), "+f"(d[9]), "+f"(d[10]), "+f"(d[11]), "+f"(d[12]), "+f"(d[13]), "+f"(d[14]), "+f"(d[15]), "+f"(d[16]), "+f"(d[17]), "+f"(d[18]), "+f"(d[19]), "+f"(d[20]), "+f"(d[21]), "+f"(d[22]), "+f"(d[23]), "+f"(d[24]), "+f"(d[25]), "+f"(d[26]), "+f"(d[27]), "+f"(d[28]), "+f"(d[29]), "+f"(d[30]), "+f"(d[31]), "+f"(d[32]), "+f"(d[33]), "+f"(d[34]), "+f"(d[35]), "+f"(d[36]), "+f"(d[37]), "+f"(d[38]), "+f"(d[39]), "+f"(d[40]), "+f"(d[41]), "+f"(d[42]), "+f"(d[43]), "+f"(d[44]), "+f"(d[45]), "+f"(d[46]), "+f"(d[47]), "+f"(d[48]), "+f"(d[49]), "+f"(d[50]), "+f"(d[51]), "+f"(d[52]), "+f"(d[53]), "+f"(d[54]), "+f"(d[55]), "+f"(d[56]), "+f"(d[57]), "+f"(d[58]), "+f"(d[59]), "+f"(d[60]), "+f"(d[61]), "+f"(d[62]), "+f"(d[63])
            : "l"(da), "l"(db), "r"(accumulate));
    }
};

template <>
struct Wgmma<256, 1> {
    static __device__ __forceinline__ void mma(float (&d)[128], uint64_t da, uint64_t db, uint32_t accumulate) {
        asm volatile(
            "{\n"
            ".reg .pred p;\n"
            "setp.ne.b32 p, %130, 0;\n"
            "wgmma.mma_async.sync.aligned.m64n256k16.f32.bf16.bf16 {%0, %1, %2, %3, %4, %5, %6, %7, %8, %9, %10, %11, %12, %13, %14, %15, %16, %17, %18, %19, %20, %21, %22, %23, %24, %25, %26, %27, %28, %29, %30, %31, %32, %33, %34, %35, %36, %37, %38, %39, %40, %41, %42, %43, %44, %45, %46, %47, %48, %49, %50, %51, %52, %53, %54, %55, %56, %57, %58, %59, %60, %61, %62, %63, %64, %65, %66, %67, %68, %69, %70, %71, %72, %73, %74, %75, %76, %77, %78, %79, %80, %81, %82, %83, %84, %85, %86, %87, %88, %89, %90, %91, %92, %93, %94, %95, %96, %97, %98, %99, %100, %101, %102, %103, %104, %105, %106, %107, %108, %109, %110, %111, %112, %113, %114, %115, %116, %117, %118, %119, %120, %121, %122, %123, %124, %125, %126, %127}, %128, %129, p, 1, 1, 0, 0;\n"
            "}\n"
            : "+f"(d[0]), "+f"(d[1]), "+f"(d[2]), "+f"(d[3]), "+f"(d[4]), "+f"(d[5]), "+f"(d[6]), "+f"(d[7]), "+f"(d[8]), "+f"(d[9]), "+f"(d[10]), "+f"(d[11]), "+f"(d[12]), "+f"(d[13]), "+f"(d[14]), "+f"(d[15]), "+f"(d[16]), "+f"(d[17]), "+f"(d[18]), "+f"(d[19]), "+f"(d[20]), "+f"(d[21]), "+f"(d[22]), "+f"(d[23]), "+f"(d[24]), "+f"(d[25]), "+f"(d[26]), "+f"(d[27]), "+f"(d[28]), "+f"(d[29]), "+f"(d[30]), "+f"(d[31]), "+f"(d[32]), "+f"(d[33]), "+f"(d[34]), "+f"(d[35]), "+f"(d[36]), "+f"(d[37]), "+f"(d[38]), "+f"(d[39]), "+f"(d[40]), "+f"(d[41]), "+f"(d[42]), "+f"(d[43]), "+f"(d[44]), "+f"(d[45]), "+f"(d[46]), "+f"(d[47]), "+f"(d[48]), "+f"(d[49]), "+f"(d[50]), "+f"(d[51]), "+f"(d[52]), "+f"(d[53]), "+f"(d[54]), "+f"(d[55]), "+f"(d[56]), "+f"(d[57]), "+f"(d[58]), "+f"(d[59]), "+f"(d[60]), "+f"(d[61]), "+f"(d[62]), "+f"(d[63]), "+f"(d[64]), "+f"(d[65]), "+f"(d[66]), "+f"(d[67]), "+f"(d[68]), "+f"(d[69]), "+f"(d[70]), "+f"(d[71]), "+f"(d[72]), "+f"(d[73]), "+f"(d[74]), "+f"(d[75]), "+f"(d[76]), "+f"(d[77]), "+f"(d[78]), "+f"(d[79]), "+f"(d[80]), "+f"(d[81]), "+f"(d[82]), "+f"(d[83]), "+f"(d[84]), "+f"(d[85]), "+f"(d[86]), "+f"(d[87]), "+f"(d[88]), "+f"(d[89]), "+f"(d[90]), "+f"(d[91]), "+f"(d[92]), "+f"(d[93]), "+f"(d[94]), "+f"(d[95]), "+f"(d[96]), "+f"(d[97]), "+f"(d[98]), "+f"(d[99]), "+f"(d[100]), "+f"(d[101]), "+f"(d[102]), "+f"(d[103]), "+f"(d[104]), "+f"(d[105]), "+f"(d[106]), "+f"(d[107]), "+f"(d[108]), "+f"(d[109]), "+f"(d[110]), "+f"(d[111]), "+f"(d[112]), "+f"(d[113]), "+f"(d[114]), "+f"(d[115]), "+f"(d[116]), "+f"(d[117]), "+f"(d[118]), "+f"(d[119]), "+f"(d[120]), "+f"(d[121]), "+f"(d[122]), "+f"(d[123]), "+f"(d[124]), "+f"(d[125]), "+f"(d[126]), "+f"(d[127])
            : "l"(da), "l"(db), "r"(accumulate));
    }
};

template <int N>
struct WgmmaRA;

template <>
struct WgmmaRA<16> {
    static __device__ __forceinline__ void mma(float (&d)[8], const uint32_t (&a)[4], uint64_t db, uint32_t accumulate) {
        asm volatile(
            "{\n"
            ".reg .pred p;\n"
            "setp.ne.b32 p, %13, 0;\n"
            "wgmma.mma_async.sync.aligned.m64n16k16.f32.f16.f16 {%0, %1, %2, %3, %4, %5, %6, %7}, {%8, %9, %10, %11}, %12, p, 1, 1, 0;\n"
            "}\n"
            : "+f"(d[0]), "+f"(d[1]), "+f"(d[2]), "+f"(d[3]), "+f"(d[4]), "+f"(d[5]), "+f"(d[6]), "+f"(d[7])
            : "r"(a[0]), "r"(a[1]), "r"(a[2]), "r"(a[3]), "l"(db), "r"(accumulate));
    }
};

template <>
struct WgmmaRA<32> {
    static __device__ __forceinline__ void mma(float (&d)[16], const uint32_t (&a)[4], uint64_t db, uint32_t accumulate) {
        asm volatile(
            "{\n"
            ".reg .pred p;\n"
            "setp.ne.b32 p, %21, 0;\n"
            "wgmma.mma_async.sync.aligned.m64n32k16.f32.f16.f16 {%0, %1, %2, %3, %4, %5, %6, %7, %8, %9, %10, %11, %12, %13, %14, %15}, {%16, %17, %18, %19}, %20, p, 1, 1, 0;\n"
            "}\n"
            : "+f"(d[0]), "+f"(d[1]), "+f"(d[2]), "+f"(d[3]), "+f"(d[4]), "+f"(d[5]), "+f"(d[6]), "+f"(d[7]), "+f"(d[8]), "+f"(d[9]), "+f"(d[10]), "+f"(d[11]), "+f"(d[12]), "+f"(d[13]), "+f"(d[14]), "+f"(d[15])
            : "r"(a[0]), "r"(a[1]), "r"(a[2]), "r"(a[3]), "l"(db), "r"(accumulate));
    }
};

template <>
struct WgmmaRA<64> {
    static __device__ __forceinline__ void mma(float (&d)[32], const uint32_t (&a)[4], uint64_t db, uint32_t accumulate) {
        asm volatile(
            "{\n"
            ".reg .pred p;\n"
            "setp.ne.b32 p, %37, 0;\n"
            "wgmma.mma_async.sync.aligned.m64n64k16.f32.f16.f16 {%0, %1, %2, %3, %4, %5, %6, %7, %8, %9, %10, %11, %12, %13, %14, %15, %16, %17, %18, %19, %20, %21, %22, %23, %24, %25, %26, %27, %28, %29, %30, %31}, {%32, %33, %34, %35}, %36, p, 1, 1, 0;\n"
            "}\n"
            : "+f"(d[0]), "+f"(d[1]), "+f"(d[2]), "+f"(d[3]), "+f"(d[4]), "+f"(d[5]), "+f"(d[6]), "+f"(d[7]), "+f"(d[8]), "+f"(d[9]), "+f"(d[10]), "+f"(d[11]), "+f"(d[12]), "+f"(d[13]), "+f"(d[14]), "+f"(d[15]), "+f"(d[16]), "+f"(d[17]), "+f"(d[18]), "+f"(d[19]), "+f"(d[20]), "+f"(d[21]), "+f"(d[22]), "+f"(d[23]), "+f"(d[24]), "+f"(d[25]), "+f"(d[26]), "+f"(d[27]), "+f"(d[28]), "+f"(d[29]), "+f"(d[30]), "+f"(d[31])
            : "r"(a[0]), "r"(a[1]), "r"(a[2]), "r"(a[3]), "l"(db), "r"(accumulate));
    }
};

template <>
struct WgmmaRA<128> {
    static __device__ __forceinline__ void mma(float (&d)[64], const uint32_t (&a)[4], uint64_t db, uint32_t accumulate) {
        asm volatile(
            "{\n"
            ".reg .pred p;\n"
            "setp.ne.b32 p, %69, 0;\n"
            "wgmma.mma_async.sync.aligned.m64n128k16.f32.f16.f16 {%0, %1, %2, %3, %4, %5, %6, %7, %8, %9, %10, %11, %12, %13, %14, %15, %16, %17, %18, %19, %20, %21, %22, %23, %24, %25, %26, %27, %28, %29, %30, %31, %32, %33, %34, %35, %36, %37, %38, %39, %40, %41, %42, %43, %44, %45, %46, %47, %48, %49, %50, %51, %52, %53, %54, %55, %56, %57, %58, %59, %60, %61, %62, %63}, {%64, %65, %66, %67}, %68, p, 1, 1, 0;\n"
            "}\n"
            : "+f"(d[0]), "+f"(d[1]), "+f"(d[2]), "+f"(d[3]), "+f"(d[4]), "+f"(d[5]), "+f"(d[6]), "+f"(d[7]), "+f"(d[8]), "+f"(d[9]), "+f"(d[10]), "+f"(d[11]), "+f"(d[12]), "+f"(d[13]), "+f"(d[14]), "+f"(d[15]), "+f"(d[16]), "+f"(d[17]), "+f"(d[18]), "+f"(d[19]), "+f"(d[20]), "+f"(d[21]), "+f"(d[22]), "+f"(d[23]), "+f"(d[24]), "+f"(d[25]), "+f"(d[26]), "+f"(d[27]), "+f"(d[28]), "+f"(d[29]), "+f"(d[30]), "+f"(d[31]), "+f"(d[32]), "+f"(d[33]), "+f"(d[34]), "+f"(d[35]), "+f"(d[36]), "+f"(d[37]), "+f"(d[38]), "+f"(d[39]), "+f"(d[40]), "+f"(d[41]), "+f"(d[42]), "+f"(d[43]), "+f"(d[44]), "+f"(d[45]), "+f"(d[46]), "+f"(d[47]), "+f"(d[48]), "+f"(d[49]), "+f"(d[50]), "+f"(d[51]), "+f"(d[52]), "+f"(d[53]), "+f"(d[54]), "+f"(d[55]), "+f"(d[56]), "+f"(d[57]), "+f"(d[58]), "+f"(d[59]), "+f"(d[60]), "+f"(d[61]), "+f"(d[62]), "+f"(d[63])
            : "r"(a[0]), "r"(a[1]), "r"(a[2]), "r"(a[3]), "l"(db), "r"(accumulate));
    }
};

}
}
```

### rq-vae-transformer_b200/rqvae/_native.py

```python
import ctypes as C
import os

import torch

_HERE = os.path.dirname(os.path.abspath(__file__))
LIB_PATH = os.environ.get("RQB200_LIB", os.path.join(os.path.dirname(_HERE), "csrc", "librqb200.so"))

OK, EINVAL, ECUDA, ENODEV, EWORKSPACE, ESTATE = 0, -1, -2, -3, -4, -5
F32, BF16, F16, E4M3 = 0, 1, 2, 3
MODE_EXACT, MODE_FAST = 0, 1
AR_NO_GRAPH, AR_NO_PDL, AR_TRACE, AR_SEQUENTIAL_PREFILL = 1, 2, 4, 32
EMB_TOK_INPUT, EMB_TOK_HEAD, EMB_NO_CUMSUM, EMB_TUPLE, EMB_CLS_PER_DEPTH = 1, 2, 4, 8, 16
_DT = {torch.float32: F32, torch.bfloat16: BF16, torch.float16: F16}

c_f32p, c_i64p, c_vp = C.c_void_p, C.c_void_p, C.c_void_p


class BlockWeights(C.Structure):
    _fields_ = [(n, C.c_void_p) for n in ("wqkv", "wproj", "w1", "w2", "bqkv", "bproj", "b1", "b2",
                                          "ln1_w", "ln1_b", "ln2_w", "ln2_b", "sqkv", "sproj", "s1", "s2")]


class ArConfig(C.Structure):
    _fields_ = [(n, C.c_int32) for n in ("embed_dim", "n_head", "n_body", "n_head_layers", "vocab", "H", "W", "D",
                                         "vocab_cond", "cond_len", "code_dim", "codebook_size", "mode", "weight_dtype",
                                         "flags", "split_qkv", "split_proj", "split_fc1", "split_fc2",
                                         "codebook_per_depth", "embed_variant")]


class ArWeights(C.Structure):
    _fields_ = [(n, C.c_void_p) for n in ("pos_emb_cond", "pos_emb_hw", "pos_emb_d", "cond_emb", "w_in", "w_head", "w_cls",
                                          "b_in", "b_head", "b_cls", "cls_ln_w", "cls_ln_b", "codebook")] + \
               [("body", C.POINTER(BlockWeights)), ("head", C.POINTER(BlockWeights))] + \
               [(n, C.c_void_p) for n in ("w_ccls", "b_ccls", "ccls_ln_w", "ccls_ln_b", "tok_emb", "s_in", "s_head", "s_cls", "s_ccls")]


class VaeConfig(C.Structure):
    _fields_ = [("ch", C.c_int32), ("n_levels", C.c_int32), ("ch_mult", C.c_int32 * 8), ("num_res_blocks", C.c_int32),
                ("n_attn_res", C.c_int32), ("attn_resolutions", C.c_int32 * 8), ("resolution", C.c_int32),
                ("z_channels", C.c_int32), ("embed_dim", C.c_int32), ("in_channels", C.c_int32), ("out_ch", C.c_int32),
                ("codebook_size", C.c_int32), ("depth", C.c_int32), ("mode", C.c_int32)]


_lib = None


class NativeError(RuntimeError):
    pass


def lib():
    global _lib
    if _lib is not None:
        return _lib
    if not os.path.exists(LIB_PATH):
        raise NativeError("rqb200: native library not found at %s -- build it with "
                          "rq-vae-transformer_b200/csrc/build.sh (or __graft_entry__.build()); there is no CPU fallback"
                          % LIB_PATH)
    L = C.CDLL(LIB_PATH)
    L.rqb200_last_error.restype = C.c_char_p
    L.rqb200_version.restype = C.c_int
    L.rqb200_device_count.restype = C.c_int
    L.rqb200_rq_quantize.argtypes = [C.c_void_p, C.c_void_p, C.c_int64, C.c_int, C.c_int, C.c_int, C.c_void_p, C.c_void_p,
                                     C.c_void_p, C.c_void_p]
    L.rqb200_rq_soft_codes.argtypes = [C.c_void_p, C.c_void_p, C.c_int64, C.c_int, C.c_int, C.c_float, C.c_void_p, C.c_void_p,
                                       C.c_void_p]
    L.rqb200_rq_embed_sum.argtypes = [C.c_void_p, C.c_void_p, C.c_int64, C.c_int, C.c_int, C.c_int, C.c_void_p, C.c_void_p]
    L.rqb200_rq_embed_depth.argtypes = L.rqb200_rq_embed_sum.argtypes
    L.rqb200_rq_quantize_depthwise.argtypes = [C.c_void_p, C.POINTER(C.c_void_p), C.POINTER(C.c_int32), C.c_int64, C.c_int, C.c_int,
                                               C.c_void_p, C.c_void_p, C.c_void_p, C.c_void_p]
    L.rqb200_dbg_rq_quantize_depthwise.argtypes = [C.c_int] + L.rqb200_rq_quantize_depthwise.argtypes
    L.rqb200_rq_embed_sum_depthwise.argtypes = [C.c_void_p, C.POINTER(C.c_void_p), C.POINTER(C.c_int32), C.c_int64, C.c_int, C.c_int,
                                                C.c_void_p, C.c_void_p]
    L.rqb200_rq_embed_depth_depthwise.argtypes = L.rqb200_rq_embed_sum_depthwise.argtypes
    L.rqb200_sample_logits.argtypes = [C.c_void_p, C.c_void_p, C.c_int, C.c_int, C.c_float, C.c_int, C.c_float, C.c_void_p,
                                       C.c_void_p]
    L.rqb200_dbg_rows_gemm.argtypes = [C.c_void_p, C.c_void_p, C.c_void_p, C.c_void_p, C.c_void_p, C.c_void_p, C.c_int, C.c_int, C.c_int64,
                                       C.c_int, C.c_int, C.c_void_p]
    L.rqb200_dbg_rq_quantize.argtypes = [C.c_int] + L.rqb200_rq_quantize.argtypes
    L.rqb200_dbg_sample_logits.argtypes = [C.c_int] + L.rqb200_sample_logits.argtypes
    L.rqb200_ar_create.restype = C.c_void_p
    L.rqb200_ar_create.argtypes = [C.POINTER(ArConfig), C.POINTER(ArWeights)]
    L.rqb200_ar_destroy.argtypes = [C.c_void_p]
    L.rqb200_ar_destroy.restype = None
    L.rqb200_ar_workspace_bytes.restype = C.c_size_t
    L.rqb200_ar_workspace_bytes.argtypes = [C.c_void_p, C.c_int]
    L.rqb200_ar_sample.argtypes = [C.c_void_p, C.c_void_p, C.c_void_p, C.c_int, C.c_int, C.c_int, C.c_float,
                                   C.POINTER(C.c_int32), C.POINTER(C.c_float), C.c_void_p, C.c_int64, C.c_void_p,
                                   C.c_void_p, C.c_void_p, C.c_void_p, C.c_size_t, C.c_void_p]
    L.rqb200_ar_sample_span.argtypes = [C.c_void_p, C.c_void_p, C.c_void_p, C.c_int, C.c_int, C.c_int, C.c_int, C.c_float,
                                        C.POINTER(C.c_int32), C.POINTER(C.c_float), C.c_void_p, C.c_int64, C.c_void_p,
                                        C.c_void_p, C.c_void_p, C.c_void_p, C.c_size_t, C.c_void_p]
    L.rqb200_ar_sample_span_cfg.argtypes = L.rqb200_ar_sample_span.argtypes + [C.c_float]
    L.rqb200_ar_sample_span_keep.argtypes = L.rqb200_ar_sample_span.argtypes + [C.c_void_p, C.c_void_p, C.c_int, C.c_float]
    L.rqb200_ar_step.argtypes = [C.c_void_p, C.c_void_p, C.c_int64, C.c_void_p, C.c_int, C.c_int, C.c_int, C.c_int, C.c_int,
                                 C.c_void_p, C.c_void_p, C.c_size_t, C.c_void_p]
    L.rqb200_ar_forward_workspace_bytes.restype = C.c_size_t
    L.rqb200_ar_forward_workspace_bytes.argtypes = [C.c_void_p, C.c_int]
    L.rqb200_ar_forward.argtypes = [C.c_void_p, C.c_void_p, C.c_void_p, C.c_int, C.c_void_p, C.c_void_p, C.c_void_p, C.c_size_t,
                                    C.c_void_p]
    L.rqb200_ar_log_prob_workspace_bytes.restype = C.c_size_t
    L.rqb200_ar_log_prob_workspace_bytes.argtypes = [C.c_void_p, C.c_int]
    L.rqb200_ar_log_prob.argtypes = L.rqb200_ar_forward.argtypes
    L.rqb200_dbg_log_prob_rows.argtypes = [C.c_void_p, C.c_int64, C.c_int, C.c_int64, C.c_void_p, C.c_void_p, C.c_void_p]
    L.rqb200_ar_trace.argtypes = [C.c_void_p, C.c_void_p, C.c_int, C.c_char_p, C.c_int]
    L.rqb200_ar_last_launches.restype = C.c_int64
    L.rqb200_ar_last_launches.argtypes = [C.c_void_p]
    L.rqb200_vae_create.restype = C.c_void_p
    L.rqb200_vae_create.argtypes = [C.POINTER(VaeConfig)]
    L.rqb200_vae_destroy.argtypes = [C.c_void_p]
    L.rqb200_vae_destroy.restype = None
    L.rqb200_vae_set_tensor.argtypes = [C.c_void_p, C.c_char_p, C.c_void_p, C.c_int, C.c_int64]
    L.rqb200_vae_finalize.argtypes = [C.c_void_p]
    L.rqb200_vae_workspace_bytes.restype = C.c_size_t
    L.rqb200_vae_workspace_bytes.argtypes = [C.c_void_p, C.c_int]
    for fn in (L.rqb200_vae_decode, L.rqb200_vae_decode_code, L.rqb200_vae_encode):
        fn.argtypes = [C.c_void_p, C.c_void_p, C.c_int, C.c_void_p, C.c_void_p, C.c_size_t, C.c_void_p]
    L.rqb200_vae_last_launches.restype = C.c_int64
    L.rqb200_vae_last_launches.argtypes = [C.c_void_p]
    L.rqb200_dbg_gemm_tc.argtypes = [C.c_void_p, C.c_void_p, C.c_void_p, C.c_void_p, C.c_void_p, C.c_int, C.c_int, C.c_void_p,
                                     C.c_int, C.c_int, C.c_int, C.c_int, C.c_int, C.c_void_p]
    L.rqb200_dbg_gemm_tc_fp8.argtypes = [C.c_void_p] * 6 + [C.c_int, C.c_int, C.c_void_p] + [C.c_int] * 4 + [C.c_void_p]
    L.rqb200_dbg_conv_tc.argtypes = [C.c_void_p, C.c_void_p, C.c_void_p, C.c_void_p, C.c_void_p, C.c_void_p, C.c_void_p, C.c_int,
                                     C.c_int, C.c_int, C.c_int, C.c_int, C.c_int, C.c_int, C.c_void_p]
    L.rqb200_dbg_conv_tc_gn.argtypes = [C.c_void_p] * 8 + [C.c_int] * 7 + [C.c_void_p]
    L.rqb200_dbg_attn_step.argtypes = [C.c_int, C.c_void_p, C.c_int] + [C.c_void_p] * 4 + [C.c_int] * 3 + [C.c_void_p] + [C.c_int] * 2 + \
                                      [C.c_void_p]
    L.rqb200_dbg_prefill_attn.argtypes = [C.c_void_p] * 4 + [C.c_int] * 5 + [C.c_void_p]
    L.rqb200_dbg_append_attn.argtypes = [C.c_void_p] * 4 + [C.c_int] * 6 + [C.c_void_p]
    L.rqb200_dbg_ln.argtypes = [C.c_int, C.c_void_p, C.c_void_p, C.c_int] + [C.c_void_p] * 6 + [C.c_int64, C.c_int, C.c_int, C.c_void_p]
    L.rqb200_dbg_act_reduce.argtypes = [C.c_void_p, C.c_int, C.c_void_p, C.c_void_p] + [C.c_int] * 3 + [C.c_void_p]
    L.rqb200_dbg_vae_conv.argtypes = [C.c_void_p, C.c_void_p, C.c_int] + [C.c_void_p] * 3 + [C.c_int] * 10 + [C.c_void_p]
    L.rqb200_dbg_groupnorm.argtypes = [C.c_int] + [C.c_void_p] * 7 + [C.c_int64] + [C.c_int] * 4 + [C.c_void_p]
    L.rqb200_dbg_cast_f16.argtypes = [C.c_void_p] * 3 + [C.c_int] * 5 + [C.c_void_p]
    L.rqb200_dbg_vae_attn.argtypes = [C.c_void_p] * 2 + [C.c_int] * 3 + [C.c_void_p]
    _lib = L
    return L


EXPORTS = ["rqb200_last_error", "rqb200_version", "rqb200_device_count", "rqb200_rq_quantize", "rqb200_rq_embed_sum",
           "rqb200_rq_embed_depth", "rqb200_rq_soft_codes", "rqb200_sample_logits", "rqb200_ar_create", "rqb200_ar_destroy",
           "rqb200_ar_workspace_bytes", "rqb200_ar_sample", "rqb200_ar_sample_span", "rqb200_ar_sample_span_cfg", "rqb200_ar_sample_span_keep", "rqb200_ar_step", "rqb200_ar_forward",
           "rqb200_ar_forward_workspace_bytes", "rqb200_ar_trace", "rqb200_ar_last_launches", "rqb200_vae_create",
           "rqb200_vae_destroy", "rqb200_vae_set_tensor", "rqb200_vae_finalize", "rqb200_vae_workspace_bytes",
           "rqb200_vae_decode", "rqb200_vae_decode_code", "rqb200_vae_encode", "rqb200_vae_last_launches",
           "rqb200_dbg_gemm_tc", "rqb200_dbg_gemm_tc_fp8", "rqb200_dbg_conv_tc", "rqb200_dbg_conv_tc_gn", "rqb200_dbg_rq_quantize", "rqb200_dbg_sample_logits",
           "rqb200_dbg_rows_gemm", "rqb200_rq_quantize_depthwise", "rqb200_rq_embed_sum_depthwise",
           "rqb200_rq_embed_depth_depthwise", "rqb200_dbg_rq_quantize_depthwise", "rqb200_ar_log_prob",
           "rqb200_ar_log_prob_workspace_bytes", "rqb200_dbg_log_prob_rows", "rqb200_dbg_attn_step", "rqb200_dbg_prefill_attn", "rqb200_dbg_append_attn",
           "rqb200_dbg_ln", "rqb200_dbg_act_reduce", "rqb200_dbg_vae_conv", "rqb200_dbg_groupnorm", "rqb200_dbg_cast_f16",
           "rqb200_dbg_vae_attn"]


def check(rc, what=""):
    if rc != 0:
        raise NativeError("rqb200 %s failed (%d): %s" % (what, rc, lib().rqb200_last_error().decode()))


def require_cuda(*tensors):
    for t in tensors:
        if t is not None and not t.is_cuda:
            raise NativeError("rqb200: tensor on %s -- this engine has no CPU path; move the model and inputs to a "
                              "CUDA device" % t.device)


def stream_ptr(device=None):
    return C.c_void_p(torch.cuda.current_stream(device).cuda_stream)


def ptr(t):
    return C.c_void_p(t.data_ptr()) if t is not None else C.c_void_p(0)


def dtype_code(t):
    return _DT[t.dtype]


def default_precision():
    return os.environ.get("RQB200_PRECISION", "auto")


def fast_dtype():
    return torch.bfloat16 if os.environ.get("RQB200_FAST_DTYPE", "fp16").lower() in ("bf16", "bfloat16") else torch.float16


def fast_weight_format():
    v = os.environ.get("RQB200_FAST_DTYPE", "fp16").lower()
    return "fp8" if v == "fp8" else ("bf16" if v in ("bf16", "bfloat16") else "fp16")


FP8_MAX = 448.0


def quantize_fp8_rows(w):
    w = w.detach().float()
    amax = w.abs().amax(dim=1)
    s = amax / torch.full_like(amax, FP8_MAX)
    s = torch.where(s > 0, s, torch.ones_like(s))
    q = (w / s[:, None]).clamp(-FP8_MAX, FP8_MAX).to(torch.float8_e4m3fn)
    return q, s


_FP8_TILE = None


def fp8_tile_order():
    global _FP8_TILE
    if _FP8_TILE is None:
        p = torch.arange(8192)
        wg, h, t, b = p // 4096, (p // 2048) % 2, (p // 16) % 128, p % 16
        kk, e, lane = 2 * h + b // 8, b % 8, t % 32
        row = 64 * wg + 16 * (t // 32) + lane // 4 + 8 * ((e // 2) % 2)
        col = 16 * kk + 2 * (lane % 4) + 8 * (e // 4) + e % 2
        _FP8_TILE = row * 64 + col
    return _FP8_TILE


def pack_fp8_tiles(q):
    N_out, K = q.shape
    if N_out % 128 or K % 64:
        raise ValueError("pack_fp8_tiles: need N %% 128 == 0 and K %% 64 == 0, got [%d, %d]" % (N_out, K))
    t = q.view(torch.uint8).reshape(N_out // 128, 128, K // 64, 64).permute(0, 2, 1, 3).reshape(-1, 8192)
    return t[:, fp8_tile_order().to(q.device)].reshape(-1).contiguous()


def unpack_fp8_tiles(packed, N_out, K):
    t = torch.empty(N_out // 128 * (K // 64), 8192, dtype=torch.uint8, device=packed.device)
    t[:, fp8_tile_order().to(packed.device)] = packed.reshape(-1, 8192)
    return t.reshape(N_out // 128, K // 64, 128, 64).permute(0, 2, 1, 3).reshape(N_out, K).view(torch.float8_e4m3fn)


def pack_fp8_weight(w):
    if w.dim() == 2:
        q, s = quantize_fp8_rows(w)
        return pack_fp8_tiles(q), s
    packed, scales = zip(*(pack_fp8_weight(w[d]) for d in range(w.shape[0])))
    return torch.cat(packed), torch.stack(scales)


def ar_engine_options():
    env = os.environ.get
    flags = 0
    flags |= AR_NO_GRAPH if env("RQB200_NO_GRAPH", "0") == "1" else 0
    flags |= AR_NO_PDL if env("RQB200_NO_PDL", "0") == "1" else 0
    flags |= AR_TRACE if env("RQB200_TRACE", "0") == "1" else 0
    flags |= AR_SEQUENTIAL_PREFILL if env("RQB200_SEQ_PREFILL", "0") == "1" else 0
    return flags


def param_fingerprint(module):
    return hash(tuple((t.data_ptr(), t._version) for t in list(module.parameters()) + list(module.buffers())))


launch_count = {"total": 0}
```

### rq-vae-transformer_b200/rqvae/models/rqvae/rqvae.py

```python
import ctypes as C
import os

import torch
from torch import nn
from torch.nn import functional as F

from ... import _native as N
from ..interfaces import Stage1Model
from .modules import Decoder, Encoder, ResnetBlock
from .quantizations import RQBottleneck


class RQVAE(Stage1Model):
    def __init__(self, *, embed_dim=64, n_embed=512, decay=0.99, loss_type="mse", latent_loss_weight=0.25,
                 bottleneck_type="rq", ddconfig=None, checkpointing=False, **kwargs):
        super().__init__()
        assert loss_type in ("mse", "l1")
        ddconfig = dict(ddconfig)
        self.ddconfig = ddconfig
        self.encoder = Encoder(**ddconfig)
        self.decoder = Decoder(**ddconfig)
        if bottleneck_type != "rq":
            raise ValueError("invalid 'bottleneck_type' (must be 'rq')")
        self.quantizer = RQBottleneck(latent_shape=kwargs["latent_shape"], code_shape=kwargs["code_shape"], n_embed=n_embed,
                                      decay=decay, shared_codebook=kwargs["shared_codebook"],
                                      restart_unused_codes=kwargs["restart_unused_codes"])
        self.code_shape = kwargs["code_shape"]
        self.embed_dim = embed_dim
        self.quant_conv = nn.Conv2d(ddconfig["z_channels"], embed_dim, 1)
        self.post_quant_conv = nn.Conv2d(embed_dim, ddconfig["z_channels"], 1)
        self.loss_type, self.latent_loss_weight = loss_type, latent_loss_weight
        self.precision = None
        self.split_fp16 = True
        self._eng = {}
        self._eng_fp = None
        self.last_launches = 0

    def _invalidate_native(self):
        for e in self._eng.values():
            N.lib().rqb200_vae_destroy(e["handle"])
        self._eng = {}

    def _apply(self, fn, *a, **k):
        self._invalidate_native()
        return super()._apply(fn, *a, **k)

    def load_state_dict(self, *a, **k):
        self._invalidate_native()
        return super().load_state_dict(*a, **k)

    def __del__(self):
        try:
            self._invalidate_native()
        except Exception:
            pass

    def _mode(self):
        p = self.precision or N.default_precision()
        return N.MODE_FAST if p == "fast" else N.MODE_EXACT

    def _engine(self, device):
        mode = self._mode()
        fp = N.param_fingerprint(self)
        if fp != self._eng_fp:
            self._invalidate_native()
            self._eng_fp = fp
        key = (str(device), mode, self.split_fp16)
        if key in self._eng:
            return self._eng[key]
        L = N.lib()
        dd = self.ddconfig
        cfg = N.VaeConfig()
        cfg.ch, cfg.n_levels, cfg.num_res_blocks = dd["ch"], len(dd["ch_mult"]), dd["num_res_blocks"]
        for i, m in enumerate(dd["ch_mult"]):
            cfg.ch_mult[i] = m
        cfg.n_attn_res = len(dd["attn_resolutions"])
        for i, r in enumerate(dd["attn_resolutions"]):
            cfg.attn_resolutions[i] = r
        cfg.resolution, cfg.z_channels, cfg.embed_dim = dd["resolution"], dd["z_channels"], self.embed_dim
        cfg.in_channels, cfg.out_ch = dd["in_channels"], dd["out_ch"]
        cfg.codebook_size, cfg.depth, cfg.mode = self.quantizer.n_embed[0], self.code_shape[-1], mode
        if os.environ.get("RQB200_GN_FUSE", "1") == "0":
            cfg.mode |= 0x100
        handle = L.rqb200_vae_create(C.byref(cfg))
        if not handle:
            raise N.NativeError("rqb200_vae_create: " + L.rqb200_last_error().decode())
        wdt = torch.float16 if mode == N.MODE_FAST else torch.float32
        keep = {}

        def reg(name, t):
            t = t.detach().contiguous()
            keep[name] = t
            N.check(L.rqb200_vae_set_tensor(handle, name.encode(), N.ptr(t), N.dtype_code(t), t.numel()), "vae_set_tensor")

        def reg_conv(name, w_oihw):
            w = w_oihw.detach().permute(0, 2, 3, 1).contiguous().float()
            if mode == N.MODE_FAST and not name.startswith("encoder.conv_in"):
                hi = w.to(torch.float16)
                reg(name, hi)
                if self.split_fp16:
                    reg(name + "_lo", (w - hi.float()).to(torch.float16))
            else:
                reg(name, w)

        sd = {k: v for k, v in self.state_dict().items()}
        for k, v in sd.items():
            if not (k.startswith("encoder.") or k.startswith("decoder.") or k.startswith("quant_conv") or
                    k.startswith("post_quant_conv")):
                continue
            N.require_cuda(v)
            if v.dim() == 4:
                if k.endswith((".q.weight", ".k.weight", ".v.weight")):
                    continue
                reg_conv(k, v)
            elif k.endswith((".q.bias", ".k.bias", ".v.bias")):
                continue
            else:
                reg(k, v.float())
        for k in [k for k in sd if k.endswith(".q.weight")]:
            base = k[:-len(".q.weight")]
            w = torch.cat([sd[base + ".q.weight"], sd[base + ".k.weight"], sd[base + ".v.weight"]], 0)
            b = torch.cat([sd[base + ".q.bias"], sd[base + ".k.bias"], sd[base + ".v.bias"]], 0)
            reg_conv(base + ".qkv.weight", w)
            reg(base + ".qkv.bias", b.float())
        tabs = self.quantizer._tables()
        if isinstance(tabs, list):
            for d, t in enumerate(tabs):
                reg("codebook.%d" % d, t.float())
        else:
            reg("codebook", tabs.float())
        N.check(L.rqb200_vae_finalize(handle), "vae_finalize")
        eng = {"handle": handle, "keep": keep, "ws": {}}
        self._eng[key] = eng
        return eng

    def _ws(self, eng, B, device):
        need = N.lib().rqb200_vae_workspace_bytes(eng["handle"], B)
        ws = eng["ws"].get("buf")
        if ws is None or ws.numel() < need:
            eng["ws"]["buf"] = ws = torch.empty(need, dtype=torch.uint8, device=device)
        return ws, need

    def _run(self, fn_name, x, out_shape):
        N.require_cuda(x)
        eng = self._engine(x.device)
        B = x.shape[0]
        out = torch.empty(out_shape, dtype=torch.float32, device=x.device)
        with torch.cuda.device(x.device):
            ws, need = self._ws(eng, B, x.device)
            fn = getattr(N.lib(), fn_name)
            N.check(fn(eng["handle"], N.ptr(x), B, N.ptr(out), N.ptr(ws), ws.numel(), N.stream_ptr(x.device)), fn_name)
        self.last_launches = N.lib().rqb200_vae_last_launches(eng["handle"])
        N.launch_count["total"] += self.last_launches
        return out

    def _latent_hw(self):
        dd = self.ddconfig
        r = dd["resolution"] // 2 ** (len(dd["ch_mult"]) - 1)
        return r

    @torch.no_grad()
    def encode(self, x):
        x = x.float().contiguous()
        r = self._latent_hw()
        return self._run("rqb200_vae_encode", x, (x.shape[0], r, r, self.embed_dim))

    @torch.no_grad()
    def decode(self, z_q):
        z_q = z_q.float().contiguous()
        dd = self.ddconfig
        return self._run("rqb200_vae_decode", z_q, (z_q.shape[0], dd["out_ch"], dd["resolution"], dd["resolution"]))

    @torch.no_grad()
    def forward(self, xs):
        z_e = self.encode(xs)
        z_q, quant_loss, code = self.quantizer(z_e)
        return self.decode(z_q), quant_loss, code

    @torch.no_grad()
    def get_codes(self, xs):
        z_e = self.encode(xs)
        _, codes = self.quantizer.quantize(self.quantizer.to_code_shape(z_e))
        return codes

    @torch.no_grad()
    def decode_code(self, code):
        assert code.shape[1:] == torch.Size(self.code_shape)
        code = code.to(torch.int64).contiguous()
        dd = self.ddconfig
        if tuple(self.quantizer.shape_divisor[:2]) != (1, 1):
            return self.decode(self.quantizer.embed_code(code))
        return self._run("rqb200_vae_decode_code", code, (code.shape[0], dd["out_ch"], dd["resolution"], dd["resolution"]))

    def get_recon_imgs(self, xs_real, xs_recon):
        return xs_real * 0.5 + 0.5, torch.clamp(xs_recon * 0.5 + 0.5, 0, 1)

    def compute_loss(self, out, quant_loss, code, xs=None, valid=False):
        loss_recon = F.mse_loss(out, xs) if self.loss_type == "mse" else F.l1_loss(out, xs)
        loss_latent = quant_loss
        if valid:
            loss_recon = loss_recon * xs.shape[0] * xs.shape[1]
            loss_latent = loss_latent * xs.shape[0]
        return {"loss_total": loss_recon + self.latent_loss_weight * loss_latent, "loss_recon": loss_recon,
                "loss_latent": loss_latent, "codes": [code]}

    def get_last_layer(self):
        return self.decoder.conv_out.weight

    @torch.no_grad()
    def get_code_emb_with_depth(self, code):
        return self.quantizer.embed_code_with_depth(code)

    @torch.no_grad()
    def decode_partial_code(self, code, code_idx, decode_type="select"):
        return self.decode(self.quantizer.embed_partial_code(code, code_idx, decode_type))

    @torch.no_grad()
    def forward_partial_code(self, xs, code_idx, decode_type="select"):
        return self.decode_partial_code(self.get_codes(xs), code_idx, decode_type)

    @torch.no_grad()
    def get_soft_codes(self, xs, temp=1.0, stochastic=False):
        z_e = self.encode(xs)
        return self.quantizer.get_soft_codes(z_e, temp=temp, stochastic=stochastic)
```

Before: 190.5.

## Replace 3-pass split-fp16 conv correction with a single FP8 E4M3 correction sweep

For split-fp16 3x3 convolutions, the two fp16 correction products (hi·lo and lo·hi) are replaced by one E4M3 wgmma sweep over packed FP8 operands. Weights get a per-tensor power-of-two scale and activations a fixed scale. Groupnorm and cast kernels now write the FP8 correction operands instead of fp16 low halves, and the main fp16 hi·hi product is accumulated on top of the rescaled correction. This is meant to cut tensor-core work and shared-memory traffic for the error-compensation terms, at the cost of lower correction precision and extra packing kernels at weight load.

```diff
diff --git a/include/rqb200.h b/include/rqb200.h
--- a/include/rqb200.h
+++ b/include/rqb200.h
@@ -167,6 +167,8 @@
                        const float* residual, float* out, int B, int H, int W, int Cin, int Cout, int ks, int out_nchw,
                        void* stream);
 
+int rqb200_pack_conv_corr(const void* w_hi, const void* w_lo, void* out, float* stat, int64_t n, int Cin, void* stream);
+
 int rqb200_dbg_conv_tc_gn(const void* X16, const void* W16, const void* X16lo, const void* W16lo, const float* bias,
                           const float* residual, float* out, double* gn_part, int B, int H, int W, int Cin, int Cout, int ks,
                           int out_nchw, void* stream);
diff --git a/rq-vae-transformer_b200/csrc/conv_tc.cu b/rq-vae-transformer_b200/csrc/conv_tc.cu
--- a/rq-vae-transformer_b200/csrc/conv_tc.cu
+++ b/rq-vae-transformer_b200/csrc/conv_tc.cu
@@ -1,3 +1,5 @@
+#include <cuda_fp8.h>
+
 #include <cstdlib>
 
 #include "kernels.h"
@@ -20,6 +22,7 @@
     int64_t m_rows;
     double* gn_part;
     int gn_chunks;
+    const float* corr_scale;
 };
 
 constexpr int CT_THREADS = 288;
@@ -270,12 +273,21 @@
                                 (PASSES == 3 || !first || j > 0) ? 1u : 0u);
 }
 
+template <int BN>
+__device__ __forceinline__ void c3_mma_corr(float (&acc)[BN / 2], uint32_t a, uint32_t b, bool first) {
+    constexpr uint32_t SBO = 10 * 128;
+#pragma unroll
+    for (int j = 0; j < 4; j++)
+        tc::WgmmaE4M3<BN>::mma(acc, tc::gmma_desc_k128(a + j * 32, SBO), tc::gmma_desc_k128(b + j * 32), (!first || j > 0) ? 1u : 0u);
+}
+
 template <int BN, int STAGES, int PASSES>
 __global__ void __launch_bounds__(CT_THREADS, 1)
 conv3x3_tc_kernel(const __grid_constant__ CUtensorMap tmA, const __grid_constant__ CUtensorMap tmB,
                   const __grid_constant__ CUtensorMap tmAlo, const __grid_constant__ CUtensorMap tmBlo, ConvTcParams p) {
     constexpr int B_BYTES = BN * 64 * 2;
     constexpr int NOPS = PASSES == 3 ? 2 : 1;
+    constexpr int SWEEPS = PASSES == 2 ? 2 : 1;
     constexpr int HSLOTS = 2;
     constexpr int SLOT_BYTES = NOPS * C3_HALO_BYTES;
     constexpr int STAGE_BYTES = NOPS * B_BYTES;
@@ -291,12 +303,17 @@
 
     const int warp = threadIdx.x >> 5, lane = threadIdx.x & 31;
     const int cslabs = p.Cin / 64;
+    const int nq = SWEEPS * cslabs;
     const int m_tiles = p.tiles_x * p.tiles_y * p.tiles_b;
     const int total = m_tiles * p.n_tiles_n;
 
     if (warp == 8 && lane == 0) {
         tc::prefetch_tmap(&tmA);
         tc::prefetch_tmap(&tmB);
+        if (PASSES != 1) {
+            tc::prefetch_tmap(&tmAlo);
+            tc::prefetch_tmap(&tmBlo);
+        }
         for (int s = 0; s < STAGES; s++) { tc::mbar_init(&full[s], 1); tc::mbar_init(&empty[s], 8); }
         for (int h = 0; h < HSLOTS; h++) { tc::mbar_init(&hfull[h], 1); tc::mbar_init(&hempty[h], 8); }
         tc::fence_barrier_init();
@@ -311,21 +328,24 @@
                 const int nt = tile % p.n_tiles_n, mt = tile / p.n_tiles_n;
                 const int tx = mt % p.tiles_x, ty = (mt / p.tiles_x) % p.tiles_y, tb = mt / (p.tiles_x * p.tiles_y);
                 const int x0 = tx * 8, y0 = ty * p.TH, b0 = tb * p.NB;
-                for (int sl = 0; sl < cslabs; sl++, hit++) {
-                    const int c0 = sl * 64;
+                for (int q = 0; q < nq; q++, hit++) {
+                    const int c0 = (q % cslabs) * 64;
+                    const bool corr = PASSES == 2 && q < cslabs;
+                    const CUtensorMap* mA = corr ? &tmAlo : &tmA;
+                    const CUtensorMap* mB = corr ? &tmBlo : &tmB;
                     for (int tap = 0; tap < 9; tap++, it++) {
                         const int s = it % STAGES;
                         tc::mbar_wait(&empty[s], ((it / STAGES) & 1) ^ 1);
                         tc::mbar_expect_tx(&full[s], STAGE_BYTES);
                         uint8_t* w = wst + s * STAGE_BYTES;
-                        tc::tma_load_2d(w, &tmB, &full[s], tap * p.Cin + c0, nt * BN, tc::L2_EVICT_LAST);
+                        tc::tma_load_2d(w, mB, &full[s], tap * p.Cin + c0, nt * BN, tc::L2_EVICT_LAST);
                         if (PASSES == 3) tc::tma_load_2d(w + B_BYTES, &tmBlo, &full[s], tap * p.Cin + c0, nt * BN, tc::L2_EVICT_LAST);
                         if (tap == 0) {
                             const int h = hit % HSLOTS;
                             tc::mbar_wait(&hempty[h], ((hit / HSLOTS) & 1) ^ 1);
                             tc::mbar_expect_tx(&hfull[h], halo_tx);
                             uint8_t* a = smem + h * SLOT_BYTES;
-                            tc::tma_load_4d(a, &tmA, &hfull[h], c0, x0 - 1, y0 - 1, b0, tc::L2_EVICT_NORMAL);
+                            tc::tma_load_4d(a, mA, &hfull[h], c0, x0 - 1, y0 - 1, b0, tc::L2_EVICT_NORMAL);
                             if (PASSES == 3) tc::tma_load_4d(a + C3_HALO_BYTES, &tmAlo, &hfull[h], c0, x0 - 1, y0 - 1, b0, tc::L2_EVICT_NORMAL);
                         }
                     }
@@ -339,12 +359,13 @@
     const int r = t & 127;
     const int rx = r % 8, ry = (r / 8) % p.TH, rb = r / (8 * p.TH);
     const uint32_t a_wg = (uint32_t)(((8 * wg / p.TH) * (p.TH + 2) + (8 * wg) % p.TH) * 10 * 128);
+    const float corr_scale = PASSES == 2 ? *p.corr_scale : 1.f;
     float acc[BN / 2];
 #pragma unroll
     for (int i = 0; i < BN / 2; i++) acc[i] = 0.f;
     uint32_t it = 0, hit = 0;
-    for (int tile = blockIdx.x; tile < total; tile += gridDim.x) {
-        for (int sl = 0; sl < cslabs; sl++, hit++) {
+    auto sweep = [&](int q0, int q1, auto mma) {
+        for (int q = q0; q < q1; q++, hit++) {
             const int h = hit % HSLOTS;
             tc::mbar_wait(&hfull[h], (hit / HSLOTS) & 1);
             const uint32_t a0 = tc::smem_u32(smem + h * SLOT_BYTES) + a_wg;
@@ -352,10 +373,9 @@
                 const int s = it % STAGES;
                 tc::mbar_wait(&full[s], (it / STAGES) & 1);
                 const uint32_t a = a0 + ((tap / 3) * 10 + tap % 3) * 128, b = tc::smem_u32(wst + s * STAGE_BYTES);
-                const bool first = sl == 0 && tap == 0;
+                const bool first = q == 0 && tap == 0;
                 tc::wgmma_fence();
-                if (p.fmt) c3_mma_kblock<BN, 1, PASSES>(acc, a, b, first);
-                else c3_mma_kblock<BN, 0, PASSES>(acc, a, b, first);
+                mma(a, b, first);
                 tc::wgmma_commit();
                 tc::wgmma_wait<1>();
                 if (!first && lane == 0) {
@@ -363,6 +383,20 @@
                     if (tap == 0) tc::mbar_arrive(&hempty[(hit - 1) % HSLOTS]);
                 }
             }
+        }
+    };
+    for (int tile = blockIdx.x; tile < total; tile += gridDim.x) {
+        if constexpr (PASSES == 2) {
+            sweep(0, cslabs, [&](uint32_t a, uint32_t b, bool first) { c3_mma_corr<BN>(acc, a, b, first); });
+            tc::wgmma_wait<0>();
+            tc::acc_fence(acc);
+#pragma unroll
+            for (int i = 0; i < BN / 2; i++) acc[i] *= corr_scale;
+            sweep(cslabs, nq, [&](uint32_t a, uint32_t b, bool) { c3_mma_kblock<BN, 0, 1>(acc, a, b, false); });
+        } else if (p.fmt) {
+            sweep(0, nq, [&](uint32_t a, uint32_t b, bool first) { c3_mma_kblock<BN, 1, PASSES>(acc, a, b, first); });
+        } else {
+            sweep(0, nq, [&](uint32_t a, uint32_t b, bool first) { c3_mma_kblock<BN, 0, PASSES>(acc, a, b, first); });
         }
         tc::wgmma_wait<0>();
         tc::acc_fence(acc);
@@ -435,7 +469,7 @@
 
 int launch_conv_tc(const void* X16, const void* W16, const void* X16lo, const void* W16lo, const float* bias,
                    const float* residual, float* out, int B, int H, int W, int Cin, int Cout, int ks, int out_nchw,
-                   cudaStream_t st, int stride, double* gn_part, int fmt) {
+                   cudaStream_t st, int stride, double* gn_part, int fmt, const float* corr_scale) {
     ConvTcParams p = {};
     p.B = B; p.H = H; p.W = W; p.Cin = Cin; p.Cout = Cout; p.ks = ks; p.stride = stride; p.fmt = fmt;
     conv_tile(H, W, ks, stride, p.TW, p.TH, p.NB);
@@ -463,6 +497,15 @@
         if (split) {
             RQB_TRY(make_tmap_4d_nhwc(&tmAlo, X16lo, (uint64_t)Cin, (uint64_t)W, (uint64_t)H, (uint64_t)B, 64, (uint32_t)p.TW + 2,
                                       (uint32_t)p.TH + 2, (uint32_t)p.NB, 1));
+            if (corr_scale != nullptr) {
+                if (fmt != 0) return fail(RQB200_EINVAL, "conv_tc: E4M3 correction operands need fp16 operands");
+                p.corr_scale = corr_scale;
+                switch (BN) {
+                    case 16: return launch_conv3x3_tc_t<16, 8, 2>(tmA, tmB, tmAlo, tmBlo, p, n_sm, st);
+                    case 64: return launch_conv3x3_tc_t<64, 8, 2>(tmA, tmB, tmAlo, tmBlo, p, n_sm, st);
+                    default: return launch_conv3x3_tc_t<128, 8, 2>(tmA, tmB, tmAlo, tmBlo, p, n_sm, st);
+                }
+            }
             switch (BN) {
                 case 16: return launch_conv3x3_tc_t<16, 8, 3>(tmA, tmB, tmAlo, tmBlo, p, n_sm, st);
                 case 64: return launch_conv3x3_tc_t<64, 4, 3>(tmA, tmB, tmAlo, tmBlo, p, n_sm, st);
@@ -515,6 +558,73 @@
     return launch_conv_tc_t<128, 6, 1>(tmA, tmB, tmA, tmB, p, n_sm, st);
 }
 
+__host__ __device__ inline int corr_sw(float amax) {
+    if (!(amax > 0.f) || amax > 3.0e38f) return 0;
+    int e;
+    const float m = frexpf(amax, &e);
+    return (m <= 0.875f ? 9 : 8) - e;
+}
+
+__device__ __forceinline__ uint32_t e4m3x4(const float (&v)[4]) {
+    const uint32_t lo = __nv_cvt_float2_to_fp8x2(make_float2(v[0], v[1]), __NV_SATFINITE, __NV_E4M3);
+    const uint32_t hi = __nv_cvt_float2_to_fp8x2(make_float2(v[2], v[3]), __NV_SATFINITE, __NV_E4M3);
+    return lo | (hi << 16);
+}
+
+__device__ __forceinline__ void store_corr4(uint8_t* out, int64_t e, int c, const float (&first)[4], const float (&second)[4]) {
+    uint8_t* p = out + 2 * e - (c & 63);
+    *reinterpret_cast<uint32_t*>(p) = e4m3x4(first);
+    *reinterpret_cast<uint32_t*>(p + 64) = e4m3x4(second);
+}
+
+__device__ __forceinline__ void act_corr4(const float* v, __half2 h0, __half2 h1, uint32_t& first, uint32_t& second) {
+    const float2 f0 = __half22float2(h0), f1 = __half22float2(h1);
+    const float hi[4] = {f0.x, f0.y, f1.x, f1.y};
+    const float lo[4] = {(v[0] - hi[0]) * 2048.f, (v[1] - hi[1]) * 2048.f, (v[2] - hi[2]) * 2048.f, (v[3] - hi[3]) * 2048.f};
+    first = e4m3x4(lo);
+    second = e4m3x4(hi);
+}
+
+__global__ void __launch_bounds__(256) amax_f16_kernel(const __half* __restrict__ x, int64_t n, float* __restrict__ stat) {
+    float m = 0.f;
+    for (int64_t i = (int64_t)blockIdx.x * 256 + threadIdx.x; i < n; i += (int64_t)gridDim.x * 256) m = fmaxf(m, fabsf(__half2float(x[i])));
+#pragma unroll
+    for (int o = 16; o; o >>= 1) m = fmaxf(m, __shfl_xor_sync(0xffffffffu, m, o));
+    if ((threadIdx.x & 31) == 0) atomicMax(reinterpret_cast<unsigned int*>(stat), __float_as_uint(m));
+}
+
+__global__ void __launch_bounds__(256) pack_corr_kernel(const __half* __restrict__ first, const __half* __restrict__ second,
+                                                        uint8_t* __restrict__ out, int64_t n, int C, float* __restrict__ stat) {
+    float sf = 2048.f, ss = 1.f;
+    if (stat != nullptr) {
+        const int sw = corr_sw(stat[0]);
+        sf = ldexpf(1.f, sw);
+        ss = ldexpf(1.f, 11 + sw);
+        if (blockIdx.x == 0 && threadIdx.x == 0) stat[1] = ldexpf(1.f, -(11 + sw));
+    }
+    for (int64_t i = (int64_t)blockIdx.x * 256 + threadIdx.x; i < n / 4; i += (int64_t)gridDim.x * 256) {
+        const int64_t e = i * 4;
+        const uint2 a = *reinterpret_cast<const uint2*>(first + e), b = *reinterpret_cast<const uint2*>(second + e);
+        const float2 a0 = __half22float2(*reinterpret_cast<const __half2*>(&a.x)), a1 = __half22float2(*reinterpret_cast<const __half2*>(&a.y));
+        const float2 b0 = __half22float2(*reinterpret_cast<const __half2*>(&b.x)), b1 = __half22float2(*reinterpret_cast<const __half2*>(&b.y));
+        const float f[4] = {a0.x * sf, a0.y * sf, a1.x * sf, a1.y * sf};
+        const float s[4] = {b0.x * ss, b0.y * ss, b1.x * ss, b1.y * ss};
+        store_corr4(out, e, (int)(e % C), f, s);
+    }
+}
+
+int launch_pack_corr(const void* first, const void* second, void* out, int64_t n, int C, float* stat, cudaStream_t st) {
+    if (n < 1 || C % 64 != 0 || n % C != 0) return fail(RQB200_EINVAL, "pack_corr: need n % C == 0 and C % 64 == 0");
+    const int gx = (int)std::min<int64_t>(ceil_div(n / 4, 256), sm_count() * 16);
+    if (stat != nullptr) {
+        if (cudaMemsetAsync(stat, 0, sizeof(float), st) != cudaSuccess) return fail(RQB200_ECUDA, "pack_corr: memset");
+        amax_f16_kernel<<<gx, 256, 0, st>>>((const __half*)first, n, stat);
+        RQB_TRY(check_launch("amax_f16"));
+    }
+    pack_corr_kernel<<<gx, 256, 0, st>>>((const __half*)first, (const __half*)second, (uint8_t*)out, n, C, stat);
+    return check_launch("pack_corr");
+}
+
 __device__ __forceinline__ void store_split4(__half* hi, __half* lo, const float (&v)[4]) {
     __half2 h0 = __floats2half2_rn(v[0], v[1]), h1 = __floats2half2_rn(v[2], v[3]);
     uint2 pk;
@@ -550,6 +660,7 @@
     fin[1] = 1.0 / sqrt(var + eps);
 }
 
+template <bool CORR>
 __global__ void __launch_bounds__(256) gn_apply_f16_kernel(const float* __restrict__ X, const double* __restrict__ part,
                                                            const float* __restrict__ gamma, const float* __restrict__ beta,
                                                            __half* __restrict__ Y, __half* __restrict__ Ylo, int HW, int C,
@@ -592,12 +703,21 @@
             l[k] = __floats2half2_rn(v[2 * k] - f.x, v[2 * k + 1] - f.y);
         }
         *reinterpret_cast<uint4*>(Yb + (size_t)i * 8) = *reinterpret_cast<uint4*>(h);
-        if (Lb) *reinterpret_cast<uint4*>(Lb + (size_t)i * 8) = *reinterpret_cast<uint4*>(l);
+        if (CORR && Lb) {
+            uint2 f, sc;
+            act_corr4(v, h[0], h[1], f.x, sc.x);
+            act_corr4(v + 4, h[2], h[3], f.y, sc.y);
+            uint8_t* cp = reinterpret_cast<uint8_t*>(Lb) + (size_t)i * 16 - (c & 63);
+            *reinterpret_cast<uint2*>(cp) = f;
+            *reinterpret_cast<uint2*>(cp + 64) = sc;
+        } else if (Lb) {
+            *reinterpret_cast<uint4*>(Lb + (size_t)i * 8) = *reinterpret_cast<uint4*>(l);
+        }
     }
 }
 
 __global__ void __launch_bounds__(256) cast_f16_kernel(const float* __restrict__ X, __half* __restrict__ Y, __half* __restrict__ Ylo,
-                                                       int B, int H, int W, int C, int upsample) {
+                                                       int B, int H, int W, int C, int upsample, int corr) {
     const int c4n = C / 4;
     const int Ho = upsample ? 2 * H : H, Wo = upsample ? 2 * W : W;
     const int64_t total4 = (int64_t)B * Ho * Wo * c4n;
@@ -608,48 +728,87 @@
         const int ix = upsample ? ox >> 1 : ox, iy = upsample ? oy >> 1 : oy;
         const float4 x = *reinterpret_cast<const float4*>(X + (((int64_t)b * H + iy) * W + ix) * C + c4 * 4);
         const float v[4] = {x.x, x.y, x.z, x.w};
-        store_split4(Y + i * 4, Ylo ? Ylo + i * 4 : nullptr, v);
+        store_split4(Y + i * 4, (Ylo && !corr) ? Ylo + i * 4 : nullptr, v);
+        if (Ylo && corr) {
+            const __half2* h = reinterpret_cast<const __half2*>(Y + i * 4);
+            uint32_t f, sc;
+            act_corr4(v, h[0], h[1], f, sc);
+            uint8_t* cp = reinterpret_cast<uint8_t*>(Ylo) + i * 8 - (c4 * 4 & 63);
+            *reinterpret_cast<uint32_t*>(cp) = f;
+            *reinterpret_cast<uint32_t*>(cp + 64) = sc;
+        }
     }
 }
 
 int launch_groupnorm_f16(const float* X, const float* gamma, const float* beta, void* Y16, void* Y16lo, double* stats_ws, int B,
-                         int HW, int C, int silu, cudaStream_t st, int fused_chunks) {
+                         int HW, int C, int silu, cudaStream_t st, int fused_chunks, int corr) {
     if (C % 128 != 0) return fail(RQB200_EINVAL, "groupnorm_f16: C % 128 != 0");
     const int nchunks = fused_chunks > 0 ? fused_chunks : (int)ceil_div(HW, 256);
     if (fused_chunks <= 0) RQB_TRY(launch_gn_stats(X, stats_ws, B, HW, C, st));
     gn_finalize_kernel<<<(unsigned)ceil_div(B * 32 * 32, 128), 128, 0, st>>>(stats_ws, B, nchunks, (double)HW * (C / 32), 1e-6);
     RQB_TRY(check_launch("gn_finalize"));
     int gx = (int)std::min<int64_t>(ceil_div((int64_t)HW * C / 8, 256), 1024);
-    gn_apply_f16_kernel<<<dim3(gx, B), 256, 0, st>>>(X, stats_ws, gamma, beta, (__half*)Y16, (__half*)Y16lo, HW, C, 1e-6f, silu, nchunks);
+    if (corr)
+        gn_apply_f16_kernel<true><<<dim3(gx, B), 256, 0, st>>>(X, stats_ws, gamma, beta, (__half*)Y16, (__half*)Y16lo, HW, C, 1e-6f, silu,
+                                                              nchunks);
+    else
+        gn_apply_f16_kernel<false><<<dim3(gx, B), 256, 0, st>>>(X, stats_ws, gamma, beta, (__half*)Y16, (__half*)Y16lo, HW, C, 1e-6f, silu,
+                                                               nchunks);
     return check_launch("gn_apply_f16");
 }
 
-int launch_cast_f16(const float* X, void* Y16, void* Y16lo, int B, int H, int W, int C, int upsample, cudaStream_t st) {
-    if (C % 4 != 0) return fail(RQB200_EINVAL, "cast_f16: C % 4 != 0");
+int launch_cast_f16(const float* X, void* Y16, void* Y16lo, int B, int H, int W, int C, int upsample, cudaStream_t st, int corr) {
+    if (C % 4 != 0 || (corr && C % 64 != 0)) return fail(RQB200_EINVAL, "cast_f16: C % 4 != 0, or C % 64 != 0 for the correction operand");
     int64_t total4 = (int64_t)B * H * W * C / 4 * (upsample ? 4 : 1);
     int gx = (int)std::min<int64_t>(ceil_div(total4, 256), sm_count() * 16);
-    cast_f16_kernel<<<gx, 256, 0, st>>>(X, (__half*)Y16, (__half*)Y16lo, B, H, W, C, upsample);
+    cast_f16_kernel<<<gx, 256, 0, st>>>(X, (__half*)Y16, (__half*)Y16lo, B, H, W, C, upsample, corr);
     return check_launch("cast_f16");
 }
 
+}
+
+namespace rqb {
+static int dbg_conv(const void* X16, const void* W16, const void* X16lo, const void* W16lo, const float* bias, const float* residual,
+                    float* out, double* gn_part, int B, int H, int W, int Cin, int Cout, int ks, int flags, cudaStream_t st) {
+    const int stride = (flags >> 8) > 1 ? (flags >> 8) : 1, fmt = (flags >> 1) & 1;
+    if (!conv_tc_supported(H, W, Cin, Cout, ks, stride, 0)) return fail(RQB200_EINVAL, "conv_tc: unsupported shape");
+    if (!(X16lo && W16lo && ks == 3 && stride == 1 && fmt == 0))
+        return launch_conv_tc(X16, W16, X16lo, W16lo, bias, residual, out, B, H, W, Cin, Cout, ks, flags & 1, st, stride, gn_part, fmt);
+    const int64_t nx = (int64_t)B * H * W * Cin, nw = (int64_t)Cout * 9 * Cin;
+    void *xc = nullptr, *wc = nullptr, *stat = nullptr;
+    if (cudaMallocAsync(&xc, nx * 2, st) != cudaSuccess || cudaMallocAsync(&wc, nw * 2, st) != cudaSuccess ||
+        cudaMallocAsync(&stat, 2 * sizeof(float), st) != cudaSuccess) {
+        if (xc) cudaFreeAsync(xc, st);
+        if (wc) cudaFreeAsync(wc, st);
+        return fail(RQB200_ECUDA, "dbg_conv_tc: cudaMallocAsync");
+    }
+    int rc = launch_pack_corr(X16lo, X16, xc, nx, Cin, nullptr, st);
+    if (rc == 0) rc = launch_pack_corr(W16, W16lo, wc, nw, Cin, (float*)stat, st);
+    if (rc == 0)
+        rc = launch_conv_tc(X16, W16, xc, wc, bias, residual, out, B, H, W, Cin, Cout, ks, flags & 1, st, stride, gn_part, fmt,
+                            (const float*)stat + 1);
+    cudaFreeAsync(xc, st);
+    cudaFreeAsync(wc, st);
+    cudaFreeAsync(stat, st);
+    return rc;
+}
 }
 
 extern "C" int rqb200_dbg_conv_tc(const void* X16, const void* W16, const void* X16lo, const void* W16lo, const float* bias,
                                   const float* residual, float* out, int B, int H, int W, int Cin, int Cout, int ks, int out_nchw,
                                   void* stream) {
-    const int stride = (out_nchw >> 8) > 1 ? (out_nchw >> 8) : 1;
-    if (!rqb::conv_tc_supported(H, W, Cin, Cout, ks, stride, 0)) return rqb::fail(RQB200_EINVAL, "conv_tc: unsupported shape");
-    return rqb::launch_conv_tc(X16, W16, X16lo, W16lo, bias, residual, out, B, H, W, Cin, Cout, ks, out_nchw & 1, (cudaStream_t)stream,
-                               stride, nullptr, (out_nchw >> 1) & 1);
+    return rqb::dbg_conv(X16, W16, X16lo, W16lo, bias, residual, out, nullptr, B, H, W, Cin, Cout, ks, out_nchw, (cudaStream_t)stream);
 }
 
 extern "C" int rqb200_dbg_conv_tc_gn(const void* X16, const void* W16, const void* X16lo, const void* W16lo, const float* bias,
                                      const float* residual, float* out, double* gn_part, int B, int H, int W, int Cin, int Cout, int ks,
                                      int out_nchw, void* stream) {
-    const int stride = (out_nchw >> 8) > 1 ? (out_nchw >> 8) : 1;
-    if (!rqb::conv_tc_supported(H, W, Cin, Cout, ks, stride, 0)) return rqb::fail(RQB200_EINVAL, "conv_tc: unsupported shape");
-    return rqb::launch_conv_tc(X16, W16, X16lo, W16lo, bias, residual, out, B, H, W, Cin, Cout, ks, out_nchw & 1, (cudaStream_t)stream,
-                               stride, gn_part, (out_nchw >> 1) & 1);
+    return rqb::dbg_conv(X16, W16, X16lo, W16lo, bias, residual, out, gn_part, B, H, W, Cin, Cout, ks, out_nchw, (cudaStream_t)stream);
+}
+
+extern "C" int rqb200_pack_conv_corr(const void* w_hi, const void* w_lo, void* out, float* stat, int64_t n, int Cin, void* stream) {
+    if (!w_hi || !w_lo || !out || !stat) return rqb::fail(RQB200_EINVAL, "pack_conv_corr: null argument");
+    return rqb::launch_pack_corr(w_hi, w_lo, out, n, Cin, stat, (cudaStream_t)stream);
 }
 
 extern "C" int rqb200_dbg_rows_gemm(const void* X16, const void* W16, const float* bias, const float* residual, float* out_f32,
diff --git a/rq-vae-transformer_b200/csrc/kernels.h b/rq-vae-transformer_b200/csrc/kernels.h
--- a/rq-vae-transformer_b200/csrc/kernels.h
+++ b/rq-vae-transformer_b200/csrc/kernels.h
@@ -62,13 +62,14 @@
 bool conv_tc_supported(int H, int W, int Cin, int Cout, int ks, int stride, int in_nchw);
 int launch_conv_tc(const void* X16, const void* W16, const void* X16lo, const void* W16lo, const float* bias,
                    const float* residual, float* out, int B, int H, int W, int Cin, int Cout, int ks, int out_nchw,
-                   cudaStream_t st, int stride = 1, double* gn_part = nullptr, int fmt = 0);
+                   cudaStream_t st, int stride = 1, double* gn_part = nullptr, int fmt = 0, const float* corr_scale = nullptr);
 bool conv_tc_gn_fusable(int H, int W, int Cout, int ks, int stride);
 int launch_rows_gemm_tc(const void* X16, const void* W16, const float* bias, const float* residual, float* out_f32, void* out_16,
                         int gelu, int fmt, int64_t M, int N_out, int K, cudaStream_t st);
 int launch_groupnorm_f16(const float* X, const float* gamma, const float* beta, void* Y16, void* Y16lo, double* stats_ws, int B,
-                         int HW, int C, int silu, cudaStream_t st, int fused_chunks = 0);
-int launch_cast_f16(const float* X, void* Y16, void* Y16lo, int B, int H, int W, int C, int upsample, cudaStream_t st);
+                         int HW, int C, int silu, cudaStream_t st, int fused_chunks = 0, int corr = 0);
+int launch_cast_f16(const float* X, void* Y16, void* Y16lo, int B, int H, int W, int C, int upsample, cudaStream_t st, int corr = 0);
+int launch_pack_corr(const void* first, const void* second, void* out, int64_t n, int C, float* stat, cudaStream_t st);
 int make_tmap_4d_nhwc(CUtensorMap* out, const void* base, uint64_t C, uint64_t W, uint64_t H, uint64_t B, uint32_t box_c,
                       uint32_t box_w, uint32_t box_h, uint32_t box_b, uint32_t stride = 1);
 
diff --git a/rq-vae-transformer_b200/csrc/vae_engine.cu b/rq-vae-transformer_b200/csrc/vae_engine.cu
--- a/rq-vae-transformer_b200/csrc/vae_engine.cu
+++ b/rq-vae-transformer_b200/csrc/vae_engine.cu
@@ -49,6 +49,8 @@
     const float* stats_buf = nullptr;
     int stats_chunks = 0;
 
+    bool corr3(int H) const { return fast && h->split && H == h->cfg.resolution; }
+
     const VTensor* get(const std::string& k, int64_t numel) {
         auto it = h->t.find(k);
         if (it == h->t.end() || it->second.numel != numel) {
@@ -59,12 +61,12 @@
     }
     void note_act(int64_t hw, int64_t c) { if (hw * c > h->max_act) h->max_act = hw * c; }
 
-    int operand(const float* x, int H, int W, int C, int slot, int upsample, Operand* o) {
+    int operand(const float* x, int H, int W, int C, int slot, int upsample, bool c3, Operand* o) {
         *o = fast ? Operand{nullptr, slot, upsample, 0} : Operand{x, -1, upsample, 0};
         if (!fast || dry) return 0;
-        return launch_cast_f16(x, h16[slot], l16[slot], B, H, W, C, upsample, st);
-    }
-    int norm(const std::string& name, const float* in, float* out, int HW, int C, int silu, Operand* o) {
+        return launch_cast_f16(x, h16[slot], l16[slot], B, H, W, C, upsample, st, c3);
+    }
+    int norm(const std::string& name, const float* in, float* out, int HW, int C, int silu, bool c3, Operand* o) {
         const VTensor* g = get(name + ".weight", C);
         const VTensor* b = get(name + ".bias", C);
         if (HW > h->max_gn_hw) h->max_gn_hw = HW;
@@ -74,7 +76,7 @@
         if (!fast) return launch_groupnorm_silu(in, (const float*)g->ptr, (const float*)b->ptr, out, gn_ws, B, HW, C, silu, st);
         const int fused = (in == stats_buf) ? stats_chunks : 0;
         stats_buf = nullptr;
-        return launch_groupnorm_f16(in, (const float*)g->ptr, (const float*)b->ptr, h16[0], l16[0], gn_ws, B, HW, C, silu, st, fused);
+        return launch_groupnorm_f16(in, (const float*)g->ptr, (const float*)b->ptr, h16[0], l16[0], gn_ws, B, HW, C, silu, st, fused, c3);
     }
     int conv(const std::string& name, const Operand& in, float* out, const float* resid, int H, int W, int Cin, int Cout, int ks,
              int stride, bool feeds_gn, int out_nchw) {
@@ -88,8 +90,17 @@
         if (w->dtype != RQB200_F16) return fail(RQB200_ESTATE, "vae fast tier: conv weights must be fp16: " + name);
         const __half* in_lo = nullptr;
         const void* w_lo = nullptr;
+        const float* corr_scale = nullptr;
         if (h->split) {
-            const VTensor* wl = get(name + ".weight_lo", (int64_t)Cout * ks * ks * Cin);
+            const VTensor* wl = nullptr;
+            if (ks == 3 && stride == 1 && corr3(Ho)) {
+                wl = get(name + ".weight_corr", (int64_t)Cout * 9 * Cin * 2);
+                const VTensor* sc = get(name + ".weight_corr_scale", 2);
+                if (!sc) return 0;
+                corr_scale = (const float*)sc->ptr + 1;
+            } else {
+                wl = get(name + ".weight_lo", (int64_t)Cout * ks * ks * Cin);
+            }
             if (!wl) return 0;
             w_lo = wl->ptr;
             in_lo = l16[in.slot];
@@ -98,19 +109,19 @@
         stats_buf = fuse ? out : nullptr;
         stats_chunks = fuse ? Ho * Wo / 32 : 0;
         return launch_conv_tc(h16[in.slot], w->ptr, in_lo, w_lo, (const float*)b->ptr, resid, out, B, Ho, Wo, Cin, Cout, ks, out_nchw, st,
-                              stride, fuse ? gn_ws : nullptr);
+                              stride, fuse ? gn_ws : nullptr, 0, corr_scale);
     }
 
     int resblock(const std::string& p, int& cur, int H, int W, int Cin, int Cout) {
         const int a = (cur + 1) & 3, b = (cur + 2) & 3, c = (cur + 3) & 3;
         Operand x;
-        RQB_TRY(norm(p + ".norm1", buf[cur], buf[a], H * W, Cin, 1, &x));
+        RQB_TRY(norm(p + ".norm1", buf[cur], buf[a], H * W, Cin, 1, corr3(H), &x));
         RQB_TRY(conv(p + ".conv1", x, buf[b], nullptr, H, W, Cin, Cout, 3, 1, true, 0));
-        RQB_TRY(norm(p + ".norm2", buf[b], buf[a], H * W, Cout, 1, &x));
+        RQB_TRY(norm(p + ".norm2", buf[b], buf[a], H * W, Cout, 1, corr3(H), &x));
         const float* res = buf[cur];
         if (Cin != Cout) {
             Operand s;
-            RQB_TRY(operand(buf[cur], H, W, Cin, 1, 0, &s));
+            RQB_TRY(operand(buf[cur], H, W, Cin, 1, 0, false, &s));
             RQB_TRY(conv(p + ".nin_shortcut", s, buf[c], nullptr, H, W, Cin, Cout, 1, 1, false, 0));
             res = buf[c];
         }
@@ -121,10 +132,10 @@
     int attnblock(const std::string& p, int& cur, int H, int W, int C) {
         const int a = (cur + 1) & 3, b = (cur + 2) & 3, c = (cur + 3) & 3;
         Operand x;
-        RQB_TRY(norm(p + ".norm", buf[cur], buf[a], H * W, C, 0, &x));
+        RQB_TRY(norm(p + ".norm", buf[cur], buf[a], H * W, C, 0, false, &x));
         RQB_TRY(conv(p + ".qkv", x, buf[b], nullptr, H, W, C, 3 * C, 1, 1, false, 0));
         if (!dry && missing.empty()) RQB_TRY(launch_vae_attn(buf[b], buf[a], B, H * W, C, st));
-        RQB_TRY(operand(buf[a], H, W, C, 0, 0, &x));
+        RQB_TRY(operand(buf[a], H, W, C, 0, 0, false, &x));
         RQB_TRY(conv(p + ".proj_out", x, buf[c], buf[cur], H, W, C, C, 1, 1, true, 0));
         cur = c;
         return 0;
@@ -140,9 +151,9 @@
         const int nl = c.n_levels, nb = c.num_res_blocks;
         int res = c.resolution >> (nl - 1), ch = c.ch * c.ch_mult[nl - 1], cur = 0;
         Operand x;
-        RQB_TRY(operand(z, res, res, c.embed_dim, 0, 0, &x));
+        RQB_TRY(operand(z, res, res, c.embed_dim, 0, 0, false, &x));
         RQB_TRY(conv("post_quant_conv", x, buf[1], nullptr, res, res, c.embed_dim, c.z_channels, 1, 1, false, 0));
-        RQB_TRY(operand(buf[1], res, res, c.z_channels, 0, 0, &x));
+        RQB_TRY(operand(buf[1], res, res, c.z_channels, 0, 0, corr3(res), &x));
         RQB_TRY(conv("decoder.conv_in", x, buf[0], nullptr, res, res, c.z_channels, ch, 3, 1, true, 0));
         RQB_TRY(resblock("decoder.mid.block_1", cur, res, res, ch, ch));
         RQB_TRY(attnblock("decoder.mid.attn_1", cur, res, res, ch));
@@ -157,13 +168,13 @@
             }
             if (lvl != 0) {
                 const int nxt = (cur + 1) & 3;
-                RQB_TRY(operand(buf[cur], res, res, ch, 1, 1, &x));
+                RQB_TRY(operand(buf[cur], res, res, ch, 1, 1, corr3(2 * res), &x));
                 RQB_TRY(conv(p + ".upsample.conv", x, buf[nxt], nullptr, res, res, ch, ch, 3, 1, true, 0));
                 cur = nxt;
                 res *= 2;
             }
         }
-        RQB_TRY(norm("decoder.norm_out", buf[cur], buf[(cur + 1) & 3], res * res, ch, 1, &x));
+        RQB_TRY(norm("decoder.norm_out", buf[cur], buf[(cur + 1) & 3], res * res, ch, 1, corr3(res), &x));
         return conv("decoder.conv_out", x, out, nullptr, res, res, ch, c.out_ch, 3, 1, false, 1);
     }
 
@@ -184,7 +195,7 @@
             }
             if (lvl != nl - 1) {
                 const int nxt = (cur + 1) & 3;
-                RQB_TRY(operand(buf[cur], res, res, ch, 1, 0, &o));
+                RQB_TRY(operand(buf[cur], res, res, ch, 1, 0, false, &o));
                 RQB_TRY(conv(p + ".downsample.conv", o, buf[nxt], nullptr, res, res, ch, ch, 3, 2, true, 0));
                 cur = nxt;
                 res /= 2;
@@ -194,9 +205,9 @@
         RQB_TRY(attnblock("encoder.mid.attn_1", cur, res, res, ch));
         RQB_TRY(resblock("encoder.mid.block_2", cur, res, res, ch, ch));
         float* zc = buf[(cur + 2) & 3];
-        RQB_TRY(norm("encoder.norm_out", buf[cur], buf[(cur + 1) & 3], res * res, ch, 1, &o));
+        RQB_TRY(norm("encoder.norm_out", buf[cur], buf[(cur + 1) & 3], res * res, ch, 1, corr3(res), &o));
         RQB_TRY(conv("encoder.conv_out", o, zc, nullptr, res, res, ch, c.z_channels, 3, 1, false, 0));
-        RQB_TRY(operand(zc, res, res, c.z_channels, 0, 0, &o));
+        RQB_TRY(operand(zc, res, res, c.z_channels, 0, 0, false, &o));
         return conv("quant_conv", o, z_e, nullptr, res, res, c.z_channels, c.embed_dim, 1, 1, false, 0);
     }
 };
@@ -352,8 +363,10 @@
 int rqb200_dbg_groupnorm(int form, const float* X, const float* gamma, const float* beta, float* Y, void* Y16, void* Y16lo,
                          double* stats_ws, int64_t ws_doubles, int B, int HW, int C, int silu, void* stream) {
     using namespace rqb;
+    const int corr = form >= 3;
+    if (corr) form -= 2;
     if (form < 0 || form > 2 || B < 1 || HW < 1 || C < 32 || C % 32 || (form > 0 && C % 128) || (form == 2 && HW % 32))
-        return fail(RQB200_EINVAL, "dbg_groupnorm: need form 0..2, B, HW >= 1, C % 32 == 0 (forms 1, 2: C % 128 == 0; form 2: HW % 32 == 0)");
+        return fail(RQB200_EINVAL, "dbg_groupnorm: need form 0..4, B, HW >= 1, C % 32 == 0 (forms 1..4: C % 128 == 0; forms 2, 4: HW % 32 == 0)");
     if (!X || !gamma || !beta || !stats_ws || (form == 0 ? !Y : !Y16))
         return fail(RQB200_EINVAL, "dbg_groupnorm: null argument");
     if (ws_doubles < 0 || (size_t)ws_doubles < groupnorm_ws_doubles(B, HW))
@@ -361,7 +374,7 @@
     if (rqb200_device_count() <= 0) return fail(RQB200_ENODEV, "dbg_groupnorm: no CUDA device");
     const cudaStream_t st = (cudaStream_t)stream;
     if (form == 0) return launch_groupnorm_silu(X, gamma, beta, Y, stats_ws, B, HW, C, silu != 0, st);
-    return launch_groupnorm_f16(X, gamma, beta, Y16, Y16lo, stats_ws, B, HW, C, silu != 0, st, form == 2 ? HW / 32 : 0);
+    return launch_groupnorm_f16(X, gamma, beta, Y16, Y16lo, stats_ws, B, HW, C, silu != 0, st, form == 2 ? HW / 32 : 0, corr);
 }
 
 int rqb200_dbg_cast_f16(const float* X, void* Y16, void* Y16lo, int B, int H, int W, int C, int upsample, void* stream) {
@@ -369,7 +382,7 @@
     if (B < 1 || H < 1 || W < 1 || C < 4) return fail(RQB200_EINVAL, "dbg_cast_f16: need B, H, W >= 1, C >= 4");
     if (!X || !Y16) return fail(RQB200_EINVAL, "dbg_cast_f16: null argument");
     if (rqb200_device_count() <= 0) return fail(RQB200_ENODEV, "dbg_cast_f16: no CUDA device");
-    return launch_cast_f16(X, Y16, Y16lo, B, H, W, C, upsample != 0, (cudaStream_t)stream);
+    return launch_cast_f16(X, Y16, Y16lo, B, H, W, C, upsample & 1, (cudaStream_t)stream, (upsample >> 1) & 1);
 }
 
 int rqb200_dbg_vae_attn(const float* qkv, float* out, int B, int HW, int C, void* stream) {
diff --git a/rq-vae-transformer_b200/csrc/wgmma.cuh b/rq-vae-transformer_b200/csrc/wgmma.cuh
--- a/rq-vae-transformer_b200/csrc/wgmma.cuh
+++ b/rq-vae-transformer_b200/csrc/wgmma.cuh
@@ -148,6 +148,51 @@
 };
 
 template <int N>
+struct WgmmaE4M3;
+
+template <>
+struct WgmmaE4M3<16> {
+    static __device__ __forceinline__ void mma(float (&d)[8], uint64_t da, uint64_t db, uint32_t accumulate) {
+        asm volatile(
+            "{\n"
+            ".reg .pred p;\n"
+            "setp.ne.b32 p, %10, 0;\n"
+            "wgmma.mma_async.sync.aligned.m64n16k32.f32.e4m3.e4m3 {%0, %1, %2, %3, %4, %5, %6, %7}, %8, %9, p, 1, 1;\n"
+            "}\n"
+            : "+f"(d[0]), "+f"(d[1]), "+f"(d[2]), "+f"(d[3]), "+f"(d[4]), "+f"(d[5]), "+f"(d[6]), "+f"(d[7])
+            : "l"(da), "l"(db), "r"(accumulate));
+    }
+};
+
+template <>
+struct WgmmaE4M3<64> {
+    static __device__ __forceinline__ void mma(float (&d)[32], uint64_t da, uint64_t db, uint32_t accumulate) {
+        asm volatile(
+            "{\n"
+            ".reg .pred p;\n"
+            "setp.ne.b32 p, %34, 0;\n"
+            "wgmma.mma_async.sync.aligned.m64n64k32.f32.e4m3.e4m3 {%0, %1, %2, %3, %4, %5, %6, %7, %8, %9, %10, %11, %12, %13, %14, %15, %16, %17, %18, %19, %20, %21, %22, %23, %24, %25, %26, %27, %28, %29, %30, %31}, %32, %33, p, 1, 1;\n"
+            "}\n"
+            : "+f"(d[0]), "+f"(d[1]), "+f"(d[2]), "+f"(d[3]), "+f"(d[4]), "+f"(d[5]), "+f"(d[6]), "+f"(d[7]), "+f"(d[8]), "+f"(d[9]), "+f"(d[10]), "+f"(d[11]), "+f"(d[12]), "+f"(d[13]), "+f"(d[14]), "+f"(d[15]), "+f"(d[16]), "+f"(d[17]), "+f"(d[18]), "+f"(d[19]), "+f"(d[20]), "+f"(d[21]), "+f"(d[22]), "+f"(d[23]), "+f"(d[24]), "+f"(d[25]), "+f"(d[26]), "+f"(d[27]), "+f"(d[28]), "+f"(d[29]), "+f"(d[30]), "+f"(d[31])
+            : "l"(da), "l"(db), "r"(accumulate));
+    }
+};
+
+template <>
+struct WgmmaE4M3<128> {
+    static __device__ __forceinline__ void mma(float (&d)[64], uint64_t da, uint64_t db, uint32_t accumulate) {
+        asm volatile(
+            "{\n"
+            ".reg .pred p;\n"
+            "setp.ne.b32 p, %66, 0;\n"
+            "wgmma.mma_async.sync.aligned.m64n128k32.f32.e4m3.e4m3 {%0, %1, %2, %3, %4, %5, %6, %7, %8, %9, %10, %11, %12, %13, %14, %15, %16, %17, %18, %19, %20, %21, %22, %23, %24, %25, %26, %27, %28, %29, %30, %31, %32, %33, %34, %35, %36, %37, %38, %39, %40, %41, %42, %43, %44, %45, %46, %47, %48, %49, %50, %51, %52, %53, %54, %55, %56, %57, %58, %59, %60, %61, %62, %63}, %64, %65, p, 1, 1;\n"
+            "}\n"
+            : "+f"(d[0]), "+f"(d[1]), "+f"(d[2]), "+f"(d[3]), "+f"(d[4]), "+f"(d[5]), "+f"(d[6]), "+f"(d[7]), "+f"(d[8]), "+f"(d[9]), "+f"(d[10]), "+f"(d[11]), "+f"(d[12]), "+f"(d[13]), "+f"(d[14]), "+f"(d[15]), "+f"(d[16]), "+f"(d[17]), "+f"(d[18]), "+f"(d[19]), "+f"(d[20]), "+f"(d[21]), "+f"(d[22]), "+f"(d[23]), "+f"(d[24]), "+f"(d[25]), "+f"(d[26]), "+f"(d[27]), "+f"(d[28]), "+f"(d[29]), "+f"(d[30]), "+f"(d[31]), "+f"(d[32]), "+f"(d[33]), "+f"(d[34]), "+f"(d[35]), "+f"(d[36]), "+f"(d[37]), "+f"(d[38]), "+f"(d[39]), "+f"(d[40]), "+f"(d[41]), "+f"(d[42]), "+f"(d[43]), "+f"(d[44]), "+f"(d[45]), "+f"(d[46]), "+f"(d[47]), "+f"(d[48]), "+f"(d[49]), "+f"(d[50]), "+f"(d[51]), "+f"(d[52]), "+f"(d[53]), "+f"(d[54]), "+f"(d[55]), "+f"(d[56]), "+f"(d[57]), "+f"(d[58]), "+f"(d[59]), "+f"(d[60]), "+f"(d[61]), "+f"(d[62]), "+f"(d[63])
+            : "l"(da), "l"(db), "r"(accumulate));
+    }
+};
+
+template <int N>
 struct WgmmaRA;
 
 template <>
diff --git a/rq-vae-transformer_b200/rqvae/_native.py b/rq-vae-transformer_b200/rqvae/_native.py
--- a/rq-vae-transformer_b200/rqvae/_native.py
+++ b/rq-vae-transformer_b200/rqvae/_native.py
@@ -11,7 +11,7 @@
 MODE_EXACT, MODE_FAST = 0, 1
 AR_NO_GRAPH, AR_NO_PDL, AR_TRACE, AR_SEQUENTIAL_PREFILL = 1, 2, 4, 32
 EMB_TOK_INPUT, EMB_TOK_HEAD, EMB_NO_CUMSUM, EMB_TUPLE, EMB_CLS_PER_DEPTH = 1, 2, 4, 8, 16
-_DT = {torch.float32: F32, torch.bfloat16: BF16, torch.float16: F16}
+_DT = {torch.float32: F32, torch.bfloat16: BF16, torch.float16: F16, torch.float8_e4m3fn: E4M3}
 
 c_f32p, c_i64p, c_vp = C.c_void_p, C.c_void_p, C.c_void_p
 
@@ -124,6 +124,7 @@
     L.rqb200_dbg_conv_tc.argtypes = [C.c_void_p, C.c_void_p, C.c_void_p, C.c_void_p, C.c_void_p, C.c_void_p, C.c_void_p, C.c_int,
                                      C.c_int, C.c_int, C.c_int, C.c_int, C.c_int, C.c_int, C.c_void_p]
     L.rqb200_dbg_conv_tc_gn.argtypes = [C.c_void_p] * 8 + [C.c_int] * 7 + [C.c_void_p]
+    L.rqb200_pack_conv_corr.argtypes = [C.c_void_p] * 4 + [C.c_int64, C.c_int, C.c_void_p]
     L.rqb200_dbg_attn_step.argtypes = [C.c_int, C.c_void_p, C.c_int] + [C.c_void_p] * 4 + [C.c_int] * 3 + [C.c_void_p] + [C.c_int] * 2 + \
                                       [C.c_void_p]
     L.rqb200_dbg_prefill_attn.argtypes = [C.c_void_p] * 4 + [C.c_int] * 5 + [C.c_void_p]
@@ -144,7 +145,7 @@
            "rqb200_ar_forward_workspace_bytes", "rqb200_ar_trace", "rqb200_ar_last_launches", "rqb200_vae_create",
            "rqb200_vae_destroy", "rqb200_vae_set_tensor", "rqb200_vae_finalize", "rqb200_vae_workspace_bytes",
            "rqb200_vae_decode", "rqb200_vae_decode_code", "rqb200_vae_encode", "rqb200_vae_last_launches",
-           "rqb200_dbg_gemm_tc", "rqb200_dbg_gemm_tc_fp8", "rqb200_dbg_conv_tc", "rqb200_dbg_conv_tc_gn", "rqb200_dbg_rq_quantize", "rqb200_dbg_sample_logits",
+           "rqb200_dbg_gemm_tc", "rqb200_dbg_gemm_tc_fp8", "rqb200_dbg_conv_tc", "rqb200_dbg_conv_tc_gn", "rqb200_pack_conv_corr", "rqb200_dbg_rq_quantize", "rqb200_dbg_sample_logits",
            "rqb200_dbg_rows_gemm", "rqb200_rq_quantize_depthwise", "rqb200_rq_embed_sum_depthwise",
            "rqb200_rq_embed_depth_depthwise", "rqb200_dbg_rq_quantize_depthwise", "rqb200_ar_log_prob",
            "rqb200_ar_log_prob_workspace_bytes", "rqb200_dbg_log_prob_rows", "rqb200_dbg_attn_step", "rqb200_dbg_prefill_attn", "rqb200_dbg_append_attn",
@@ -199,6 +200,15 @@
     s = torch.where(s > 0, s, torch.ones_like(s))
     q = (w / s[:, None]).clamp(-FP8_MAX, FP8_MAX).to(torch.float8_e4m3fn)
     return q, s
+
+
+def pack_conv_corr(w_hi, w_lo):
+    w_hi, w_lo = w_hi.contiguous(), w_lo.contiguous()
+    out = torch.empty(2 * w_hi.numel(), dtype=torch.float8_e4m3fn, device=w_hi.device)
+    stat = torch.empty(2, dtype=torch.float32, device=w_hi.device)
+    check(lib().rqb200_pack_conv_corr(ptr(w_hi), ptr(w_lo), ptr(out), ptr(stat), w_hi.numel(), w_hi.shape[-1],
+                                      stream_ptr(w_hi.device)), "pack_conv_corr")
+    return out, stat
 
 
 _FP8_TILE = None
diff --git a/rq-vae-transformer_b200/rqvae/models/rqvae/rqvae.py b/rq-vae-transformer_b200/rqvae/models/rqvae/rqvae.py
--- a/rq-vae-transformer_b200/rqvae/models/rqvae/rqvae.py
+++ b/rq-vae-transformer_b200/rqvae/models/rqvae/rqvae.py
@@ -99,7 +99,12 @@
                 hi = w.to(torch.float16)
                 reg(name, hi)
                 if self.split_fp16:
-                    reg(name + "_lo", (w - hi.float()).to(torch.float16))
+                    lo = (w - hi.float()).to(torch.float16)
+                    reg(name + "_lo", lo)
+                    if w.shape[1] == 3 and ".downsample." not in name and w.shape[-1] % 64 == 0:
+                        corr, stat = N.pack_conv_corr(hi, lo)
+                        reg(name + "_corr", corr)
+                        reg(name + "_corr_scale", stat)
             else:
                 reg(name, w)
 
```

Result: faster. 194.3 (median of 6 runs) (+2.0%).
